# Zhijian-Mei/py-debruijn

Measured on AMD Instinct MI355X. Metric: k-mers/s hashed+graph-built at k=31, higher is better.
Workload: dtype u64

## Files before the change

py-debruijn_amd/_dbg.py:

```python
from __future__ import annotations

import ctypes as C
import os

import numpy as np

_HERE = os.path.dirname(os.path.abspath(__file__))
LIB_PATH = os.environ.get("DBG_LIB") or os.path.join(_HERE, "libdbg_hip.so")

DBG_OK, DBG_E_ARG, DBG_E_HIP, DBG_E_ALPHABET, DBG_E_CAPACITY, DBG_E_NOMEM = 0, -1, -2, -3, -4, -5
F_INDEG, F_KEEP_MASK, F_KEEP_SHIFT, F_BRANCH, F_PULLED = 0x01, 0x1E, 1, 0x20, 0x40
NO_NODE = 0xFFFFFFFF
ABI_VERSION = 6

SYMBOLS = (
    "dbg_create", "dbg_destroy", "dbg_last_error", "dbg_abi_version", "dbg_set_option", "dbg_set_reads", "dbg_set_reads_fasta",
    "dbg_set_reads_fasta_file", "dbg_fasta_ingest_stats", "dbg_set_reads_device",
    "dbg_synth_reads", "dbg_reads_checksum", "dbg_copy_reads", "dbg_reads_device", "dbg_build", "dbg_refine_edge_order", "dbg_export_orders",
    "dbg_get_alphabet", "dbg_export_keepmask", "dbg_export_dict_order",
    "dbg_prune", "dbg_remove_tips",
    "dbg_mark_pull_reads", "dbg_walk", "dbg_get_sizes", "dbg_get_stats", "dbg_get_counter", "dbg_export_nodes", "dbg_export_keys_hi",
    "dbg_export_succ",
    "dbg_export_csr", "dbg_export_pull_ranks", "dbg_export_pull_reads", "dbg_export_contigs",
    "dbg_export_contig_index", "dbg_export_contig_text", "dbg_device_views", "dbg_shard_extract", "dbg_shard_bucket_counts", "dbg_shard_record_layout", "dbg_shard_build", "dbg_shard_answer", "dbg_shard_apply",
    "dbg_import_graph", "dbg_device_keys_hi",
    "dbg_support_read_scores", "dbg_export_sorted_fasta", "dbg_build_multipass", "dbg_part_count", "dbg_part_sizes", "dbg_export_part", "dbg_part_device_views",
    "dbg_shard_build_multipass", "dbg_shard_build_multipass_from", "dbg_shard_extract_part", "dbg_part_queries", "dbg_part_answer", "dbg_part_apply", "dbg_multipass_finish",
    "dbg_export_marked", "dbg_part_keys_hi", "dbg_take_reads",
    "dbg_part_prune", "dbg_part_select", "dbg_part_gather", "dbg_part_mark", "dbg_part_clear", "dbg_part_cross_targets",
    "dbg_part_segments", "dbg_part_pflags", "dbg_scan_reads_for_keys", "dbg_set_orders", "dbg_part_segment_text",
    "dbg_build_from_walk", "dbg_build_from_walks",
)


class Sizes(C.Structure):
    _fields_ = [("k", C.c_int32), ("abi_version", C.c_int32)] + [
        (n, C.c_uint64) for n in (
            "n_reads", "n_bytes", "n_kmer_instances", "n_edge_instances", "table_capacity", "n_nodes", "n_edges",
            "n_branch", "n_pulled", "n_pull_reads", "n_starts", "n_contigs", "contig_chars", "tip_rounds",
            "contigs_materialised", "max_degree")]

    def as_dict(self):
        return {n: getattr(self, n) for n, _ in self._fields_}


class Stats(C.Structure):
    _fields_ = [(n, C.c_double) for n in (
        "ms_startbits", "ms_table_init", "ms_count", "ms_compact", "ms_succ", "ms_csr", "ms_build_total", "ms_prune",
        "ms_tips", "ms_pull_reads", "ms_walk", "ms_h2d", "ms_extract", "ms_partition")] + [
        (n, C.c_uint64) for n in ("count_launches", "n_records", "n_buckets", "n_queries")]

    def as_dict(self):
        return {n: getattr(self, n) for n, _ in self._fields_}


class IngestStats(C.Structure):
    _fields_ = [(n, C.c_uint64) for n in (
        "bytes_read", "chunks", "chunk_bytes", "peak_device_bytes", "n_reads", "n_bases")] + [
        (n, C.c_double) for n in ("ms_total", "ms_io_wait", "ms_h2d", "ms_parse")]

    def as_dict(self):
        return {n: getattr(self, n) for n, _ in self._fields_}


class WalkBlock(C.Structure):
    _fields_ = [("src", C.c_void_p), ("contigs", C.c_void_p), ("n", C.c_uint64)]


COUNTERS = ("extract_presplit_fallbacks", "extract_presplit_rehists", "resolve_direct_hits", "resolve_keyed")


class DbgError(RuntimeError):
    def __init__(self, code, msg):
        super().__init__(f"dbg error {code}: {msg}")
        self.code = code


class AlphabetError(DbgError, ValueError):
    pass


_lib = None


def load_library():
    global _lib
    if _lib is not None:
        return _lib
    if not os.path.exists(LIB_PATH):
        raise OSError(f"{LIB_PATH} not found: build it with py-debruijn_amd/csrc/build.sh "
                      f"(there is no CPU fallback for the device path)")
    try:
        import torch
    except ImportError:
        pass
    lib = C.CDLL(LIB_PATH)
    H = C.c_void_p
    u64p, u32p, u8p = C.POINTER(C.c_uint64), C.POINTER(C.c_uint32), C.POINTER(C.c_uint8)
    vp = C.c_void_p
    sig = {
        "dbg_create": (C.c_int, [C.c_int, C.POINTER(H)]),
        "dbg_destroy": (None, [H]),
        "dbg_last_error": (C.c_char_p, [H]),
        "dbg_abi_version": (C.c_int, []),
        "dbg_set_option": (C.c_int, [H, C.c_char_p, C.c_int64]),
        "dbg_set_reads": (C.c_int, [H, vp, vp, C.c_uint64]),
        "dbg_set_reads_fasta": (C.c_int, [H, vp, C.c_uint64]),
        "dbg_set_reads_fasta_file": (C.c_int, [H, C.c_char_p, C.c_uint64, C.c_uint64, C.c_uint64]),
        "dbg_fasta_ingest_stats": (C.c_int, [H, C.POINTER(IngestStats)]),
        "dbg_set_reads_device": (C.c_int, [H, vp, C.c_uint64, vp, C.c_uint64]),
        "dbg_synth_reads": (C.c_int, [H, C.c_uint64, C.c_uint64, C.c_uint64, C.c_uint64, C.c_uint32, C.c_uint32]),
        "dbg_reads_checksum": (C.c_int, [H, u64p]),
        "dbg_copy_reads": (C.c_int, [H, vp, vp]),
        "dbg_build": (C.c_int, [H, C.c_int, C.c_uint64]),
        "dbg_refine_edge_order": (C.c_int, [H]),
        "dbg_export_orders": (C.c_int, [H, vp, vp]),
        "dbg_get_alphabet": (C.c_int, [H, vp, C.POINTER(C.c_int), C.POINTER(C.c_int)]),
        "dbg_export_keepmask": (C.c_int, [H, vp]),
        "dbg_prune": (C.c_int, [H, C.c_double]),
        "dbg_remove_tips": (C.c_int, [H]),
        "dbg_mark_pull_reads": (C.c_int, [H]),
        "dbg_walk": (C.c_int, [H, C.c_int, C.c_uint64]),
        "dbg_get_sizes": (C.c_int, [H, C.POINTER(Sizes)]),
        "dbg_get_stats": (C.c_int, [H, C.POINTER(Stats)]),
        "dbg_get_counter": (C.c_int, [H, C.c_char_p, C.POINTER(C.c_uint64)]),
        "dbg_export_nodes": (C.c_int, [H, vp, vp, vp, vp]),
        "dbg_export_keys_hi": (C.c_int, [H, vp]),
        "dbg_export_dict_order": (C.c_int, [H, vp]),
        "dbg_export_succ": (C.c_int, [H, vp]),
        "dbg_export_csr": (C.c_int, [H, vp, vp, vp]),
        "dbg_export_pull_ranks": (C.c_int, [H, vp]),
        "dbg_export_pull_reads": (C.c_int, [H, vp]),
        "dbg_export_contigs": (C.c_int, [H, vp, vp, vp, vp, vp]),
        "dbg_export_contig_index": (C.c_int, [H, vp, vp, vp, vp]),
        "dbg_export_contig_text": (C.c_int, [H, C.c_uint64, vp, C.c_uint64]),
        "dbg_device_views": (C.c_int, [H] + [C.POINTER(vp)] * 5),
        "dbg_shard_extract": (C.c_int, [H, C.c_int, C.c_int, u64p, C.POINTER(vp), C.POINTER(vp), C.POINTER(vp)]),
        "dbg_shard_bucket_counts": (C.c_int, [H, u64p]),
        "dbg_shard_record_layout": (C.c_int, [H, C.POINTER(C.c_int), C.POINTER(C.c_int)]),
        "dbg_shard_build": (C.c_int, [H, C.c_int, C.c_int, C.c_int, vp, vp, vp, u64p, u64p, u64p, u64p, C.POINTER(vp), u64p, C.c_int]),
        "dbg_shard_answer": (C.c_int, [H, vp, C.c_uint64, vp]),
        "dbg_build_multipass": (C.c_int, [H, C.c_int, C.c_int]),
        "dbg_export_sorted_fasta": (C.c_int, [H, vp, vp, C.c_uint64, u64p]),
        "dbg_support_read_scores": (C.c_int, [H, vp, vp, C.c_uint64, vp, vp, vp, vp, C.c_uint64, vp, vp]),
        "dbg_part_count": (C.c_int, [H, C.POINTER(C.c_int)]),
        "dbg_shard_build_multipass": (C.c_int, [H, C.c_int, C.c_int, C.c_int, C.c_int, vp, vp, vp, C.c_int, u64p, u64p, u64p]),
        "dbg_shard_build_multipass_from": (C.c_int, [H, C.c_int, C.c_int, C.c_int, C.c_int, C.c_int, vp, vp, vp, C.c_int, u64p, u64p, u64p]),
        "dbg_shard_extract_part": (C.c_int, [H, C.c_int, C.c_int, C.c_int, C.c_int, u64p, C.POINTER(C.c_void_p), C.POINTER(C.c_void_p), C.POINTER(C.c_void_p)]),
        "dbg_part_queries": (C.c_int, [H, C.c_int, u64p, u64p, C.POINTER(vp)]),
        "dbg_part_answer": (C.c_int, [H, C.c_int, vp, C.c_uint64, vp]),
        "dbg_part_apply": (C.c_int, [H, C.c_int, C.c_int, vp]),
        "dbg_multipass_finish": (C.c_int, [H]),
# ... 650 lines not shown
```

py-debruijn_amd/csrc/dbg_hip.hip:

```cpp
#include <hip/hip_runtime.h>

#include <algorithm>
#include <chrono>
#include <cstdlib>
#include <cstdio>
#include <cstring>
#include <string>
#include <vector>

#include <cerrno>
#include <fcntl.h>
#include <sys/stat.h>
#include <unistd.h>

#include <rocprim/device/device_radix_sort.hpp>

#include "../../include/dbg.h"
#include "dbg_device.h"
#include "dbg_sk.h"
#include "dbg_sk2.h"
#include "dbg_sk3.h"
#include "dbg_wsk2.h"
#include "dbg_generic.h"
#include "dbg_genref.h"
// ... 58 lines not shown
    uint8_t *d_fsorder = nullptr;
    bool order_exact = false;
    uint32_t *d_succ = nullptr;
    bool nodes_in_arena = false;
    bool csr_built = false;
    uint64_t *d_rowptr = nullptr;
    uint32_t *d_col = nullptr, *d_ecnt = nullptr;
    bool dense_pending = false;
    uint32_t *d_rowptr32 = nullptr;
    void *d_stamps_st = nullptr;
    int stamps_st_bytes = 0;

    bool pruned = false, tipped = false;
    uint64_t n_branch = 0, n_pulled = 0, tip_rounds = 0;
    uint64_t *d_pull_rank = nullptr;

    uint8_t *d_read_flags = nullptr;
    uint64_t n_pull_reads = 0;
    bool pull_reads_done = false;

    uint64_t n_starts = 0, n_contigs = 0, contig_chars = 0;
    bool starts_known = false;
    struct { const uint64_t *w0 = nullptr, *w1 = nullptr; const void *st = nullptr; int st_bytes = 0;
             const uint64_t *b_start = nullptr, *b_cnt = nullptr; bool valid = false; } sk_src;
    uint64_t *d_ctg_off = nullptr;
    char *d_ctg_chars = nullptr;
    uint64_t *d_ctg_score = nullptr, *d_ctg_stamp = nullptr;
    uint32_t *d_ctg_seq = nullptr;
    uint32_t *d_ctg_start = nullptr;
    uint32_t *d_lift = nullptr;
    int lift_levels = 0;
    bool walked = false;
    bool walk_final = false;
    bool walk_indexed = false;
    uint64_t walk_jump_min = 1ull << 14;

    int D = 4, sym_bits = 2, n_sym = 0;
    bool alpha_known = false, is_dna = true;
    uint8_t alphabet[32] = {0};
    uint8_t *d_lut = nullptr;
    char *d_alpha = nullptr;
    uint32_t *d_keepmask = nullptr;
    uint8_t *d_rank_mc = nullptr, *d_rank_fs = nullptr;

    int engine = 0;
    int bucket_bits = 0;
    int lds_slots = 4096;
    int phase_limit = 0;
    int est_scale_pct = 100;
    int wide_engine = 1;
    int count_kernel_u64 = 3;
    int stamp64 = 0;
    int resolve_sorted = 0;
    int resolve_direct = 1;
    int resolve_count = 0;
    uint64_t resolve_direct_hits = 0, resolve_keyed = 0;
    int wcount_kernel = 2;
    int count_kernel = 2;

    struct Buf {
        void *p = nullptr;
        uint64_t bytes = 0;
    };
    Buf ar_rec[2][3], ar_q[2][3], ar_node[8], ar_misc[MISC_SLOTS], ar_csr[4], ar_dir, ar_l2, ar_scan, ar_shard[6], ar_walk[3], ar_wide[6], ar_refine[4], ar_tips[4], ar_part[4][3] ;
    int sk_T = 0, sk_l1 = 0, sk_l2 = 0, sk_nb2 = 0 , sk_cap = 0;
    bool refine_streaming = false;
    int target_distinct = 0;
    int shard_stamp64 = 0;
    int extract_generic = 0;
    int extract_presplit = DBG_EXTRACT_PRESPLIT;
    uint64_t presplit_rehists = 0;
    uint64_t presplit_fallbacks = 0;
    uint64_t sk_n_ranges = 0, sk_n_buckets = 0;
    SkGeom sk_geom{};
    void *shard_state = nullptr;
    void *multipass = nullptr;
    bool dropping_parts = false;
    dbg *spare_part = nullptr;
    bool wide_owner = false;
    bool borrowed_stream = false;
    bool arena_freed = false;
    std::vector<uint64_t> host_seg_cnt;
    std::vector<uint64_t> host_scpre;
    uint64_t shard_node_limit = 0;
    bool partial_graph = false;
    uint64_t *d_btab = nullptr;
    uint64_t btab_cap = 0;
    struct NkBlock {
        uint64_t n_src = 0, n_reads = 0;
        uint32_t *next = nullptr, *z = nullptr, *start = nullptr;
    };
    bool nk_graph = false;
    uint64_t nk_reads = 0, nk_bytes = 0;
    std::vector<NkBlock> nk_blocks;
    uint8_t *d_nk_read_flags = nullptr;

    dbg_stats_t stats{};
    dbg_ingest_stats_t ingest{};
};

struct ShardState {
    int n_shards = 0, my_shard = 0, shard_bits = 0, k = 0;
    std::vector<uint64_t> q_start, q_cnt;
    uint64_t n_remote = 0;
    uint64_t n_kmer_inst_local = 0;
    std::vector<uint64_t> l1_counts;
    int rec_words = 1, rec_stamp_bytes = 4;
};
static ShardState &shard_of(dbg *h);
static void multipass_free(dbg *h);
static void drop_spare_part(dbg *h);

static int buf_ensure(dbg *h, dbg::Buf &b, uint64_t bytes) {
    if (bytes == 0) bytes = 16;
    if (b.bytes >= bytes) return DBG_OK;
    if (b.p) { (void)hipFreeAsync(b.p, h->stream); h->arena_freed = true; }
    b.p = nullptr;
    b.bytes = 0;
    static const bool trace = getenv("DBG_TRACE_ALLOC") != nullptr;
    const auto t_alloc = std::chrono::steady_clock::now();
    hipError_t e = hipMallocAsync(&b.p, bytes, h->stream);
    if (trace) {
        const double ms = std::chrono::duration<double, std::milli>(std::chrono::steady_clock::now() - t_alloc).count();
        if (ms > 5.0) fprintf(stderr, "[dbg] hipMallocAsync(%.3f GB) took %.1f ms (buffer %p of handle %p)\n", bytes / 1e9, ms, (void *)&b, (void *)h);
    }
    if (e != hipSuccess) {
        (void)hipGetLastError();
        (void)hipStreamSynchronize(h->stream);
        hipMemPool_t pool;
        if (hipDeviceGetDefaultMemPool(&pool, h->device) == hipSuccess) (void)hipMemPoolTrimTo(pool, 0);
        e = hipMallocAsync(&b.p, bytes, h->stream);
    }
    if (e != hipSuccess) {
        (void)hipGetLastError();
        h->err = std::string("hipMallocAsync(") + std::to_string(bytes) + "): " + hipGetErrorString(e);
        b.p = nullptr;
        return DBG_E_NOMEM;
    }
    b.bytes = bytes;
    return DBG_OK;
}
static void buf_free(dbg *h, dbg::Buf &b) {
    if (b.p) { (void)hipFreeAsync(b.p, h->stream); h->arena_freed = true; }
    b.p = nullptr;
    b.bytes = 0;
}
static void pool_trim(dbg *h) {
    if (!h->arena_freed) return;
    (void)hipStreamSynchronize(h->stream);
    hipMemPool_t pool;
    if (hipDeviceGetDefaultMemPool(&pool, h->device) == hipSuccess) (void)hipMemPoolTrimTo(pool, 0);
    (void)hipGetLastError();
    h->arena_freed = false;
}

#define HIPCHK(h, call)                                                                      \
    do {                                                                                     \
        hipError_t e_ = (call);                                                              \
        if (e_ != hipSuccess) {                                                              \
            (h)->err = std::string(#call) + ": " + hipGetErrorString(e_);                    \
            return e_ == hipErrorOutOfMemory ? DBG_E_NOMEM : DBG_E_HIP;                      \
        }                                                                                    \
    } while (0)

#define CHK(expr)                 \
    do {                          \
        int rc_ = (expr);         \
        if (rc_ != DBG_OK) return rc_; \
    } while (0)

template <class T>
static int dev_alloc(dbg *h, T **p, uint64_t count) {
    *p = nullptr;
    if (count == 0) count = 1;
    HIPCHK(h, hipMalloc((void **)p, count * sizeof(T)));
    return DBG_OK;
}
template <class T>
static void dev_free(T *&p) {
    if (p) (void)hipFree(p);
    p = nullptr;
}

static inline unsigned grid_for(uint64_t n, unsigned block) { return (unsigned)((n + block - 1) / block); }

struct Timer {
    hipEvent_t a = nullptr, b = nullptr;
    hipStream_t s;
    explicit Timer(hipStream_t st) : s(st) {
        (void)hipEventCreate(&a);
        (void)hipEventCreate(&b);
        (void)hipEventRecord(a, s);
    }
    double stop() {
        (void)hipEventRecord(b, s);
        (void)hipEventSynchronize(b);
        float ms = 0;
        (void)hipEventElapsedTime(&ms, a, b);
        return ms;
    }
    ~Timer() {
        (void)hipEventDestroy(a);
        (void)hipEventDestroy(b);
    }
};

constexpr int SCAN_ITEMS = 16;
constexpr int SCAN_TILE = 256 * SCAN_ITEMS;

template <class F>
__global__ __launch_bounds__(256) void k_scan_reduce(uint64_t n, F f, uint64_t *partial) {
    uint64_t base = (uint64_t)blockIdx.x * SCAN_TILE + (uint64_t)threadIdx.x * SCAN_ITEMS;
    uint64_t s = 0;
#pragma unroll
    for (int i = 0; i < SCAN_ITEMS; ++i)
        if (base + i < n) s += f(base + i);
    uint64_t tot;
    (void)block_exscan_256(s, &tot);
    if (threadIdx.x == 0) partial[blockIdx.x] = tot;
}

__global__ __launch_bounds__(256) void k_scan_partials(uint64_t *partial, uint64_t nblk, uint64_t *total) {
    uint64_t carry = 0;
    for (uint64_t base = 0; base < nblk; base += 256) {
        uint64_t i = base + threadIdx.x;
        uint64_t v = i < nblk ? partial[i] : 0;
        uint64_t tot;
        uint64_t ex = block_exscan_256(v, &tot);
        if (i < nblk) partial[i] = carry + ex;
        carry += tot;
    }
    if (threadIdx.x == 0) *total = carry;
}

template <class F, class OutT>
__global__ __launch_bounds__(256) void k_scan_write(uint64_t n, F f, const uint64_t *partial, OutT *out) {
    uint64_t base = (uint64_t)blockIdx.x * SCAN_TILE + (uint64_t)threadIdx.x * SCAN_ITEMS;
    uint64_t v[SCAN_ITEMS];
    uint64_t s = 0;
#pragma unroll
    for (int i = 0; i < SCAN_ITEMS; ++i) {
        v[i] = (base + i < n) ? f(base + i) : 0;
        s += v[i];
    }
    uint64_t tot;
    uint64_t run = partial[blockIdx.x] + block_exscan_256(s, &tot);
#pragma unroll
    for (int i = 0; i < SCAN_ITEMS; ++i) {
        if (base + i < n) out[base + i] = (OutT)run;
        run += v[i];
    }
}

template <class F, class OutT>
static int exclusive_scan(dbg *h, uint64_t n, F f, OutT *out, uint64_t *h_total) {
    uint64_t nblk = (n + SCAN_TILE - 1) / SCAN_TILE;
    if (nblk == 0) nblk = 1;
    CHK(buf_ensure(h, h->ar_scan, (nblk + 1) * 8));
    uint64_t *partial = (uint64_t *)h->ar_scan.p;
    uint64_t *d_total = partial + nblk;
    hipLaunchKernelGGL(HIP_KERNEL_NAME(k_scan_reduce<F>), dim3((unsigned)nblk), dim3(256), 0, h->stream, n, f, partial);
    hipLaunchKernelGGL(k_scan_partials, dim3(1), dim3(256), 0, h->stream, partial, nblk, d_total);
    hipLaunchKernelGGL(HIP_KERNEL_NAME(k_scan_write<F, OutT>), dim3((unsigned)nblk), dim3(256), 0, h->stream, n, f,
                       partial, out);
    if (!h_total) return DBG_OK;
    hipError_t e = hipMemcpyAsync(h_total, d_total, 8, hipMemcpyDeviceToHost, h->stream);
    if (e == hipSuccess) e = hipStreamSynchronize(h->stream);
    if (e != hipSuccess) {
        h->err = std::string("exclusive_scan: ") + hipGetErrorString(e);
        return DBG_E_HIP;
    }
    return DBG_OK;
}

template <class F>
static int reduce_sum(dbg *h, uint64_t n, F f, uint64_t *h_total) {
    uint64_t nblk = (n + SCAN_TILE - 1) / SCAN_TILE;
    if (nblk == 0) nblk = 1;
    CHK(buf_ensure(h, h->ar_scan, (nblk + 1) * 8));
    uint64_t *partial = (uint64_t *)h->ar_scan.p;
    hipLaunchKernelGGL(HIP_KERNEL_NAME(k_scan_reduce<F>), dim3((unsigned)nblk), dim3(256), 0, h->stream, n, f, partial);
    hipLaunchKernelGGL(k_scan_partials, dim3(1), dim3(256), 0, h->stream, partial, nblk, partial + nblk);
    hipError_t e = hipMemcpyAsync(h_total, partial + nblk, 8, hipMemcpyDeviceToHost, h->stream);
    if (e == hipSuccess) e = hipStreamSynchronize(h->stream);
    if (e != hipSuccess) {
        h->err = std::string("reduce_sum: ") + hipGetErrorString(e);
        return DBG_E_HIP;
    }
// ... 1026 lines not shown
                                                   uint64_t n_nodes, int levels, char *chars) {
    const uint64_t c = (uint64_t)blockIdx.x * blockDim.x + threadIdx.x;
    if (c >= n_chars) return;
    uint64_t lo = 0, hi = n_ctg;
    while (hi - lo > 1) {
        const uint64_t mid = (lo + hi) >> 1;
        if (ctg_off[mid] <= c) lo = mid; else hi = mid;
    }
    const uint64_t j = c - ctg_off[lo];
    uint32_t x = ctg_start[lo];
    if (j < (uint64_t)g.k) { chars[c] = g.char_at(x, (int)j); return; }
    uint64_t d = j - (uint64_t)g.k + 1;
    for (int l = 0; l < levels && d; ++l, d >>= 1)
        if (d & 1) x = up[(uint64_t)l * n_nodes + x];
    chars[c] = g.sym_char(g.last_code(x));
}

static const char *const kPartialGraph =
    "this handle holds one shard of a multi-GPU build: gather the shards first (multi_gpu.gather_graph / dbg_import_graph)";
static int nk_mark_contigs(dbg *h);
static void free_build(dbg *h) {
    multipass_free(h);
    dev_free(h->d_tab); dev_free(h->d_occ);
    if (h->nodes_in_arena) {
        h->d_keys = nullptr; h->d_stamps = nullptr; h->d_cnt = nullptr; h->d_flags = nullptr;
        h->d_order = nullptr; h->d_succ = nullptr; h->d_deg = nullptr; h->d_keys_hi = nullptr;
        h->nodes_in_arena = false;
    }
    dev_free(h->d_btab);
    h->btab_cap = 0;
    dev_free(h->d_keys_hi);
    dev_free(h->d_fsorder);
    h->order_exact = false;
    dev_free(h->d_keepmask); dev_free(h->d_rank_mc); dev_free(h->d_rank_fs);
    h->D = 4; h->sym_bits = 2;
    dev_free(h->d_keys); dev_free(h->d_stamps); dev_free(h->d_cnt); dev_free(h->d_flags);
    dev_free(h->d_order); dev_free(h->d_succ); dev_free(h->d_deg);
    h->d_rowptr = nullptr; h->d_col = nullptr; h->d_ecnt = nullptr;
    h->d_rowptr32 = nullptr; h->d_stamps_st = nullptr; h->stamps_st_bytes = 0;
    h->dense_pending = false;
    h->csr_built = false;
    h->d_pull_rank = nullptr;
    dev_free(h->d_read_flags);
    dev_free(h->d_ctg_off); dev_free(h->d_ctg_chars); dev_free(h->d_ctg_score); dev_free(h->d_ctg_stamp);
    dev_free(h->d_ctg_seq); dev_free(h->d_ctg_start); dev_free(h->d_lift);
    h->lift_levels = 0;
    h->partial_graph = false;
    h->sk_src.valid = false;
    h->k = 0; h->cap = 0; h->n_nodes = h->n_edges = 0;
    h->pruned = h->tipped = h->pull_reads_done = h->walked = h->walk_indexed = false;
    h->n_branch = h->n_pulled = h->tip_rounds = h->n_pull_reads = 0;
    h->n_starts = h->n_contigs = h->contig_chars = 0;
    h->starts_known = false;
    h->n_kmer_inst = h->n_edge_inst = 0;
    for (auto &b : h->nk_blocks) { dev_free(b.next); dev_free(b.z); dev_free(b.start); }
    h->nk_blocks.clear();
    dev_free(h->d_nk_read_flags);
    h->nk_graph = false;
    h->nk_reads = h->nk_bytes = 0;
}

static void free_reads(dbg *h) {
    if (h->own_bases) dev_free(h->d_bases);
    if (h->own_offsets) dev_free(h->d_offsets);
    h->d_bases = nullptr; h->d_offsets = nullptr;
    h->own_bases = h->own_offsets = false;
    dev_free(h->d_startbits);
    dev_free(h->d_lut); dev_free(h->d_alpha);
    h->alpha_known = false;
    h->n_bytes = h->n_reads = 0;
}

extern "C" int dbg_abi_version(void) { return DBG_ABI_VERSION; }

extern "C" int dbg_create(int device, dbg_t **out) {
    if (!out) return DBG_E_ARG;
    *out = nullptr;
    int n = 0;
    if (hipGetDeviceCount(&n) != hipSuccess || device < 0 || device >= n) return DBG_E_HIP;
    dbg *h = new (std::nothrow) dbg();
    if (!h) return DBG_E_NOMEM;
    h->device = device;
    if (hipSetDevice(device) != hipSuccess || hipStreamCreate(&h->stream) != hipSuccess ||
        hipMalloc((void **)&h->d_scalars, 128 * sizeof(uint64_t)) != hipSuccess) {
        delete h;
        return DBG_E_HIP;
    }
    {
        hipMemPool_t pool;
        if (hipDeviceGetDefaultMemPool(&pool, device) == hipSuccess) {
            uint64_t keep = ~0ull;
            (void)hipMemPoolSetAttribute(pool, hipMemPoolAttrReleaseThreshold, &keep);
        }
        (void)hipGetLastError();
    }
    *out = h;
    return DBG_OK;
}

extern "C" void dbg_destroy(dbg_t *h) {
    if (!h) return;
    (void)hipSetDevice(h->device);
    (void)hipStreamSynchronize(h->stream);
    h->dropping_parts = true;
    free_build(h);
    if (h->spare_part) { dbg_destroy(h->spare_part); h->spare_part = nullptr; }
    free_reads(h);
    for (auto &lvl : h->ar_rec) for (auto &b : lvl) buf_free(h, b);
    for (auto &lvl : h->ar_q) for (auto &b : lvl) buf_free(h, b);
    for (auto &b : h->ar_node) buf_free(h, b);
    for (auto &b : h->ar_misc) buf_free(h, b);
    for (auto &b : h->ar_csr) buf_free(h, b);
    buf_free(h, h->ar_dir);
    buf_free(h, h->ar_l2);
    for (auto &b : h->ar_shard) buf_free(h, b);
    for (auto &b : h->ar_walk) buf_free(h, b);
    for (auto &b : h->ar_wide) buf_free(h, b);
    for (auto &b : h->ar_refine) buf_free(h, b);
    for (auto &b : h->ar_tips) buf_free(h, b);
    for (auto &lvl : h->ar_part) for (auto &b : lvl) buf_free(h, b);
    buf_free(h, h->ar_scan);
    dev_free(h->d_scalars);
    delete (ShardState *)h->shard_state;
    (void)hipStreamSynchronize(h->stream);
    if (!h->borrowed_stream) (void)hipStreamDestroy(h->stream);
    delete h;
}

extern "C" const char *dbg_last_error(const dbg_t *h) { return h ? h->err.c_str() : "null handle"; }

static int make_startbits(dbg *h) {
    Timer t(h->stream);
    dev_free(h->d_startbits);
    h->startbits_words = (h->n_bytes + 1 + 31) / 32 + SB_WORDS + 2;
    CHK(dev_alloc(h, &h->d_startbits, h->startbits_words));
    HIPCHK(h, hipMemsetAsync(h->d_startbits, 0, h->startbits_words * 4, h->stream));
    hipLaunchKernelGGL(k_startbits, dim3(grid_for(h->n_reads + 1, 256)), dim3(256), 0, h->stream, h->d_offsets,
                       h->n_reads, h->d_startbits);
    HIPCHK(h, hipGetLastError());
    h->stats.ms_startbits = t.stop();
    return DBG_OK;
}

extern "C" int dbg_set_reads(dbg_t *h, const char *bases, const uint64_t *offsets, uint64_t n_reads) {
    if (!h || !offsets || (n_reads && !bases && offsets[n_reads] != 0)) return DBG_E_ARG;
    HIPCHK(h, hipSetDevice(h->device));
    if (offsets[0] != 0) { h->err = "offsets[0] must be 0"; return DBG_E_ARG; }
    for (uint64_t i = 0; i < n_reads; ++i)
        if (offsets[i + 1] < offsets[i]) { h->err = "offsets must be non-decreasing"; return DBG_E_ARG; }
    free_build(h);
    free_reads(h);
    const uint64_t nb = offsets[n_reads];
    Timer t(h->stream);
    CHK(dev_alloc(h, &h->d_bases, nb + 64));
    h->own_bases = true;
    CHK(dev_alloc(h, &h->d_offsets, n_reads + 1));
    h->own_offsets = true;
    if (nb) HIPCHK(h, hipMemcpyAsync(h->d_bases, bases, nb, hipMemcpyHostToDevice, h->stream));
    HIPCHK(h, hipMemcpyAsync(h->d_offsets, offsets, (n_reads + 1) * 8, hipMemcpyHostToDevice, h->stream));
    h->stats.ms_h2d = t.stop();
    h->n_bytes = nb;
    h->n_reads = n_reads;
    return make_startbits(h);
}

extern "C" int dbg_set_reads_fasta(dbg_t *h, const char *text, uint64_t n_text) {
    if (!h || (n_text && !text)) return DBG_E_ARG;
    HIPCHK(h, hipSetDevice(h->device));
    free_build(h);
    free_reads(h);
    char *d_text = nullptr;
    uint32_t *bits = nullptr, *word_rank = nullptr, *len = nullptr;
    uint64_t *line_start = nullptr, *read_idx = nullptr, *byte_off = nullptr;
    uint8_t *is_read = nullptr;
    auto cleanup = [&]() {
        dev_free(d_text); dev_free(bits); dev_free(word_rank); dev_free(len); dev_free(line_start); dev_free(read_idx);
        dev_free(byte_off); dev_free(is_read);
    };
    int rc = DBG_OK;
    uint64_t n_lines = 0, n_reads = 0, n_bases = 0;
    do {
        Timer t(h->stream);
        if ((rc = dev_alloc(h, &d_text, n_text + 64)) != DBG_OK) break;
        if (n_text && hipMemcpyAsync(d_text, text, n_text, hipMemcpyHostToDevice, h->stream) != hipSuccess) { h->err = "H2D copy failed"; rc = DBG_E_HIP; break; }
        h->stats.ms_h2d = t.stop();
        const uint64_t n_words = (n_text + 31) / 32;
        if ((rc = dev_alloc(h, &bits, n_words)) != DBG_OK) break;
        if ((rc = dev_alloc(h, &word_rank, n_words)) != DBG_OK) break;
        if (n_words) {
            hipLaunchKernelGGL(k_fa_mark, dim3(grid_for(n_words, 256)), dim3(256), 0, h->stream, d_text, n_text, bits);
            if ((rc = exclusive_scan(h, n_words, PopcWords{bits}, word_rank, &n_lines)) != DBG_OK) break;
        }
        if ((rc = dev_alloc(h, &line_start, n_lines)) != DBG_OK) break;
        if ((rc = dev_alloc(h, &is_read, n_lines)) != DBG_OK) break;
        if ((rc = dev_alloc(h, &len, n_lines)) != DBG_OK) break;
        if ((rc = dev_alloc(h, &read_idx, n_lines)) != DBG_OK) break;
        if ((rc = dev_alloc(h, &byte_off, n_lines)) != DBG_OK) break;
        if (n_lines) {
            hipLaunchKernelGGL(k_fa_line_starts, dim3(grid_for(n_words, 256)), dim3(256), 0, h->stream, bits, word_rank, n_words,
                               line_start);
            hipLaunchKernelGGL(k_fa_lines, dim3(grid_for(n_lines, 256)), dim3(256), 0, h->stream, d_text, n_text, line_start,
                               n_lines, is_read, len);
            if ((rc = exclusive_scan(h, n_lines, ByteSet{is_read}, read_idx, &n_reads)) != DBG_OK) break;
            if ((rc = exclusive_scan(h, n_lines, U32At{len}, byte_off, &n_bases)) != DBG_OK) break;
        }
        if ((rc = dev_alloc(h, &h->d_bases, n_bases + 64)) != DBG_OK) break;
        h->own_bases = true;
// ... 600 lines not shown
    uint32_t *occ = nullptr, *eocc = nullptr, *word_rank = nullptr;
    unsigned long long *estamp = nullptr;
    auto cleanup = [&]() { dev_free(nodes); dev_free(edges); dev_free(occ); dev_free(eocc); dev_free(word_rank); dev_free(estamp); };
    int rc = DBG_OK;
    do {
        if ((rc = dev_alloc(h, &nodes, cap)) != DBG_OK) break;
        if ((rc = dev_alloc(h, &edges, cap)) != DBG_OK) break;
        if ((rc = dev_alloc(h, &occ, cap / 32)) != DBG_OK) break;
        if ((rc = dev_alloc(h, &eocc, cap / 32)) != DBG_OK) break;
        (void)hipMemsetAsync(occ, 0, cap / 8, h->stream);
        (void)hipMemsetAsync(eocc, 0, cap / 8, h->stream);
        (void)hipMemsetAsync(h->d_scalars, 0, 64 * 8, h->stream);
        hipLaunchKernelGGL(k_g_init_tables, dim3(grid_for(cap, 256)), dim3(256), 0, h->stream, nodes, edges, cap);
        if (h->n_bytes) {
            const unsigned grid = (unsigned)std::min<uint64_t>((h->n_bytes + 255) / 256, 1u << 16);
            hipLaunchKernelGGL(k_g_insert, dim3(grid), dim3(256), 0, h->stream, h->d_bases, h->n_bytes, h->d_startbits, k,
                               h->d_lut, nodes, occ, edges, eocc, cap - 1, (unsigned long long *)h->d_scalars);
        }
        uint64_t sc[4] = {0, 0, 0, 0};
        if (hipMemcpyAsync(sc, h->d_scalars, 32, hipMemcpyDeviceToHost, h->stream) != hipSuccess ||
            hipStreamSynchronize(h->stream) != hipSuccess) { h->err = "generic count failed"; rc = DBG_E_HIP; break; }
        if (sc[0] & STATUS_TABLE_FULL) { h->err = "generic engine: hash table full"; rc = DBG_E_CAPACITY; break; }
        h->n_kmer_inst = sc[1];
        h->n_edge_inst = sc[2];
        h->stats.ms_count = t_count.stop();
        h->stats.count_launches = 1;
        Timer t_c(h->stream);
        const uint64_t n_words = cap / 32;
        if ((rc = dev_alloc(h, &word_rank, n_words)) != DBG_OK) break;
        uint64_t n = 0;
        if ((rc = exclusive_scan(h, n_words, PopcWords{occ}, word_rank, &n)) != DBG_OK) break;
        h->n_nodes = n;
        if ((rc = dev_alloc(h, &h->d_keys, n)) != DBG_OK) break;
        if ((rc = dev_alloc(h, &h->d_stamps, n)) != DBG_OK) break;
        if ((rc = dev_alloc(h, &h->d_flags, n)) != DBG_OK) break;
        if ((rc = dev_alloc(h, &h->d_cnt, n * GEN_D)) != DBG_OK) break;
        if ((rc = dev_alloc(h, &h->d_succ, n * GEN_D)) != DBG_OK) break;
        if ((rc = dev_alloc(h, &h->d_deg, n)) != DBG_OK) break;
        if ((rc = dev_alloc(h, &h->d_keepmask, n)) != DBG_OK) break;
        if ((rc = dev_alloc(h, &h->d_rank_mc, n * GEN_D)) != DBG_OK) break;
        if ((rc = dev_alloc(h, &h->d_rank_fs, n * GEN_D)) != DBG_OK) break;
        if ((rc = dev_alloc(h, &estamp, n * GEN_D)) != DBG_OK) break;
        if (n) {
            (void)hipMemsetAsync(h->d_cnt, 0, n * GEN_D * 4, h->stream);
            (void)hipMemsetAsync(h->d_succ, 0xFF, n * GEN_D * 4, h->stream);
            (void)hipMemsetAsync(estamp, 0xFF, n * GEN_D * 8, h->stream);
            (void)hipMemsetAsync(h->d_keepmask, 0, n * 4, h->stream);
            hipLaunchKernelGGL(k_g_gather, dim3(grid_for(n_words, 256)), dim3(256), 0, h->stream, nodes, occ, word_rank, n_words,
                               h->d_keys, h->d_stamps, h->d_flags);
            hipLaunchKernelGGL(k_g_edges, dim3(grid_for(cap, 256)), dim3(256), 0, h->stream, edges, cap, nodes, cap - 1, k,
                               h->d_cnt, h->d_succ, estamp, (unsigned long long *)h->d_scalars);
            hipLaunchKernelGGL(k_g_rank, dim3(grid_for(n, 256)), dim3(256), 0, h->stream, n, h->d_cnt, estamp, h->d_rank_mc,
                               h->d_rank_fs, h->d_deg);
        }
        if (hipMemcpyAsync(sc, h->d_scalars, 8, hipMemcpyDeviceToHost, h->stream) != hipSuccess ||
            hipStreamSynchronize(h->stream) != hipSuccess) { h->err = "generic graph assembly failed"; rc = DBG_E_HIP; break; }
        if (sc[0] & STATUS_SUCC_MISSING) { h->err = "internal: edge endpoint missing from the node table"; rc = DBG_E_HIP; break; }
        h->stats.ms_succ = t_c.stop();
        h->order_exact = true;
    } while (0);
    cleanup();
    return rc;
}

extern "C" int dbg_set_option(dbg_t *h, const char *name, int64_t value) {
    if (!h || !name) return DBG_E_ARG;
    const std::string n(name);
    if (n == "engine" && (value == 0 || value == 1)) { h->engine = (int)value; return DBG_OK; }
    if (n == "bucket_bits" && value >= 0 && value <= SK_BUCKET_BITS) { h->bucket_bits = (int)value; return DBG_OK; }
    if (n == "lds_slots" && (value == 2048 || value == 4096)) { h->lds_slots = (int)value; return DBG_OK; }
    if (n == "phase_limit" && value >= 0 && value <= 5) { h->phase_limit = (int)value; return DBG_OK; }
    if (n == "estimate_scale_pct" && value >= 1 && value <= 1000) { h->est_scale_pct = (int)value; return DBG_OK; }
    if (n == "target_distinct" && value >= 0 && value <= 4096) { h->target_distinct = (int)value; return DBG_OK; }
    if (n == "shard_stamp64" && (value == 0 || value == 1)) { h->shard_stamp64 = (int)value; return DBG_OK; }
    if (n == "extract_generic" && (value == 0 || value == 1)) { h->extract_generic = (int)value; return DBG_OK; }
    if (n == "extract_presplit" && value >= 0 && value <= SK_PS_MAX_F0) { h->extract_presplit = (int)value; return DBG_OK; }
    if (n == "refine_streaming" && (value == 0 || value == 1)) { h->refine_streaming = value != 0; return DBG_OK; }
    if (n == "walk_jump_min_nodes" && value >= 0) { h->walk_jump_min = (uint64_t)value; return DBG_OK; }
    if (n == "wide_engine" && (value == 0 || value == 1)) { h->wide_engine = (int)value; return DBG_OK; }
    if (n == "count_kernel" && value >= 1 && value <= 3) { h->count_kernel = (int)value; return DBG_OK; }
    if (n == "stamp64" && (value == 0 || value == 1)) { h->stamp64 = (int)value; return DBG_OK; }
    if (n == "resolve_sorted" && value >= 0 && value <= 2) { h->resolve_sorted = (int)value; return DBG_OK; }
    if (n == "resolve_direct" && (value == 0 || value == 1)) { h->resolve_direct = (int)value; return DBG_OK; }
    if (n == "resolve_count" && (value == 0 || value == 1)) { h->resolve_count = (int)value; return DBG_OK; }
    if (n == "wcount_kernel" && (value == 1 || value == 2)) { h->wcount_kernel = (int)value; return DBG_OK; }
    if (n == "count_kernel_u64" && value >= 1 && value <= 3) { h->count_kernel_u64 = (int)value; return DBG_OK; }
    if (n == "shard_node_limit" && value >= 0 && value < (1ll << 29)) { h->shard_node_limit = (uint64_t)value; return DBG_OK; }
    h->err = "unknown option or value out of range: " + n;
    return DBG_E_ARG;
}

static int build_wide_once(dbg *h, int k, uint64_t table_capacity_hint, bool packed, bool *overflow) {
    if (h->n_bytes >= (1ull << 43)) { h->err = "reads too large for the 44-bit positions of the table's protocol word"; return DBG_E_CAPACITY; }
    uint64_t want = table_capacity_hint;
    if (!want) {
        uint64_t inst = 0;
        CHK(reduce_sum(h, h->n_reads, KmerInstances{h->d_offsets, (uint64_t)k}, &inst));
        want = (uint64_t)((double)(inst + 1) / 0.7);
    }
    const uint64_t cap = std::max<uint64_t>(1024, (want + 1023) / 1024 * 1024);
    const uint64_t pk_words = (h->n_bytes + 31) / 32, n_occ = cap / 32;
    uint64_t *pk = nullptr;
    WSlot *tab = nullptr;
    uint32_t *tcnt = nullptr, *word_rank = nullptr;
    uint8_t *occ = nullptr;
    auto cleanup = [&]() {};
    int rc = DBG_OK;
    uint64_t sc[4] = {0, 0, 0, 0};
    do {
        Timer t(h->stream);
        if ((rc = buf_ensure(h, h->ar_wide[0], (pk_words + 3) * 8)) != DBG_OK) break;
        if ((rc = buf_ensure(h, h->ar_wide[1], cap * sizeof(WSlot))) != DBG_OK) break;
        if (!packed && (rc = buf_ensure(h, h->ar_wide[2], cap * 16)) != DBG_OK) break;
        if ((rc = buf_ensure(h, h->ar_wide[3], cap)) != DBG_OK) break;
        if ((rc = buf_ensure(h, h->ar_wide[4], n_occ * 4)) != DBG_OK) break;
        pk = (uint64_t *)h->ar_wide[0].p;
        tab = (WSlot *)h->ar_wide[1].p;
        tcnt = packed ? nullptr : (uint32_t *)h->ar_wide[2].p;
        occ = (uint8_t *)h->ar_wide[3].p;
        word_rank = (uint32_t *)h->ar_wide[4].p;
        (void)hipMemsetAsync(pk + pk_words, 0, 3 * 8, h->stream);
        hipLaunchKernelGGL(k_wtab_init, dim3(grid_for(cap, 256)), dim3(256), 0, h->stream, tab, cap);
        if (tcnt) (void)hipMemsetAsync(tcnt, 0, cap * 16, h->stream);
        (void)hipMemsetAsync(occ, 0, cap, h->stream);
        (void)hipMemsetAsync(h->d_scalars, 0, 64 * 8, h->stream);
        if (pk_words)
            hipLaunchKernelGGL(k_wpack, dim3(grid_for(pk_words, 256)), dim3(256), 0, h->stream, h->d_bases, h->n_bytes,
                               pk_words, pk);
        h->stats.ms_table_init = t.stop();
        Timer tc(h->stream);
        const uint64_t tiles = (h->n_bytes + TILE - 1) / TILE;
        if (tiles)
            hipLaunchKernelGGL(k_wcount, dim3((unsigned)tiles), dim3(256), 0, h->stream, h->d_bases, h->n_bytes,
                               h->d_startbits, k, pk, tab, tcnt, cap, occ, (unsigned long long *)h->d_scalars);
        h->stats.count_launches = tiles ? 1 : 0;
        hipError_t e = hipMemcpyAsync(sc, h->d_scalars, 32, hipMemcpyDeviceToHost, h->stream);
        h->stats.ms_count = tc.stop();
        if (e != hipSuccess || hipGetLastError() != hipSuccess) { h->err = "k_wcount failed"; rc = DBG_E_HIP; break; }
        if (sc[0] & STATUS_BAD_BASE) { h->err = "reads hold a byte outside ACGT"; rc = DBG_E_ALPHABET; break; }
        if (sc[0] & STATUS_TABLE_FULL) { h->err = "hash table capacity exceeded"; rc = DBG_E_CAPACITY; break; }
        if (sc[0] & STATUS_WIDE_COUNTER16) { *overflow = true; rc = DBG_E_CAPACITY; h->err = "successor counter overflow"; break; }
        h->n_kmer_inst = sc[1];
        h->n_edge_inst = sc[2];

        Timer tg(h->stream);
        uint64_t total = 0;
        if ((rc = exclusive_scan(h, n_occ, OccBytes32{occ}, word_rank, &total)) != DBG_OK) break;
        if (total >= 0xFFFFFFFFull) { h->err = "more than 2^32-1 nodes"; rc = DBG_E_CAPACITY; break; }
        h->n_nodes = total;
        if ((rc = buf_ensure(h, h->ar_node[0], total * 8)) != DBG_OK) break;
        if ((rc = buf_ensure(h, h->ar_node[1], total * 8)) != DBG_OK) break;
        if ((rc = buf_ensure(h, h->ar_node[2], total * 16)) != DBG_OK) break;
        if ((rc = buf_ensure(h, h->ar_node[3], total)) != DBG_OK) break;
        if ((rc = buf_ensure(h, h->ar_node[4], total)) != DBG_OK) break;
        if ((rc = buf_ensure(h, h->ar_node[5], total * 16)) != DBG_OK) break;
        if ((rc = buf_ensure(h, h->ar_node[6], total)) != DBG_OK) break;
        if ((rc = buf_ensure(h, h->ar_wide[5], total * 8)) != DBG_OK) break;
        h->d_keys = (uint64_t *)h->ar_node[0].p;
        h->d_stamps = (uint64_t *)h->ar_node[1].p;
        h->d_cnt = (uint32_t *)h->ar_node[2].p;
        h->d_flags = (uint8_t *)h->ar_node[3].p;
        h->d_order = (uint8_t *)h->ar_node[4].p;
        h->d_succ = (uint32_t *)h->ar_node[5].p;
        h->d_deg = (uint8_t *)h->ar_node[6].p;
        h->d_keys_hi = (uint64_t *)h->ar_wide[5].p;
        h->nodes_in_arena = true;
// ... 717 lines not shown
                               base_chr, per_score, h->d_stamps, h->d_ctg_off, h->d_ctg_score, h->d_ctg_stamp, h->d_ctg_seq,
                               ctg_start);
            hipError_t e = hipStreamSynchronize(h->stream);
            if (e != hipSuccess) { h->err = std::string("walk index: ") + hipGetErrorString(e); rc = DBG_E_HIP; break; }
            h->walk_indexed = true;
            if (n_chr > max_chars) break;
            const uint64_t longest = h->n_nodes + (uint64_t)h->k;
            int levels = 1;
            while ((1ull << levels) <= longest) ++levels;
            if (n_ctg && (uint64_t)levels * h->n_nodes * 4 <= (8ull << 30)) {
                if ((rc = dev_alloc(h, &h->d_ctg_chars, n_chr)) != DBG_OK) break;
                if ((rc = dev_alloc(h, &lift, (uint64_t)levels * h->n_nodes)) != DBG_OK) break;
                const dim3 ngrid(grid_for(h->n_nodes, 256));
                hipLaunchKernelGGL(HIP_KERNEL_NAME(k_lift_init<G>), ngrid, dim3(256), 0, h->stream, h->n_nodes, g, lift);
                for (int l = 1; l < levels; ++l)
                    hipLaunchKernelGGL(k_lift_step, ngrid, dim3(256), 0, h->stream, h->n_nodes, lift + (uint64_t)(l - 1) * h->n_nodes,
                                       lift + (uint64_t)l * h->n_nodes);
                hipLaunchKernelGGL(HIP_KERNEL_NAME(k_text_fill<G>), dim3(grid_for(n_chr, 256)), dim3(256), 0, h->stream, n_chr, g,
                                   h->d_ctg_off, n_ctg, ctg_start, lift, h->n_nodes, levels, h->d_ctg_chars);
                text_done = true;
            }
        }
        if (!text_done) {
            if ((rc = dev_alloc(h, &h->d_ctg_chars, n_chr)) != DBG_OK) break;
            launch(1);
        }
        if (hipGetLastError() != hipSuccess) { h->err = "walk pass 1 launch failed"; rc = DBG_E_HIP; break; }
        hipError_t e = hipStreamSynchronize(h->stream);
        if (e != hipSuccess) { h->err = std::string("walk: ") + hipGetErrorString(e); rc = DBG_E_HIP; break; }
        h->walked = true;
        h->walk_indexed = true;
    } while (0);
    cleanup();
    h->stats.ms_walk = t.stop();
    return rc;
}

extern "C" int dbg_walk(dbg_t *h, int final_mode, uint64_t max_chars) {
    if (!h || !h->pruned) { if (h) h->err = "dbg_prune must run first"; return DBG_E_ARG; }
    HIPCHK(h, hipSetDevice(h->device));
    if (h->D == GEN_D) return walk_impl(h, gen_view(h), final_mode, max_chars);
    return walk_impl(h, dna_view(h), final_mode, max_chars);
}

extern "C" int dbg_get_sizes(dbg_t *h, dbg_sizes_t *o) {
    if (!h || !o) return DBG_E_ARG;
    if (h->k && h->n_nodes && !h->starts_known) {
        HIPCHK(h, hipSetDevice(h->device));
        CHK(ensure_starts(h));
    }
    memset(o, 0, sizeof(*o));
    o->k = h->k;
    o->abi_version = DBG_ABI_VERSION;
    o->n_reads = h->n_reads + h->nk_reads;
    o->n_bytes = h->n_bytes + h->nk_bytes;
    o->n_kmer_instances = h->n_kmer_inst;
    o->n_edge_instances = h->n_edge_inst;
    o->table_capacity = h->cap;
    o->n_nodes = h->n_nodes;
    o->n_edges = h->n_edges;
    o->n_branch = h->n_branch;
    o->n_pulled = h->n_pulled;
    o->n_pull_reads = h->n_pull_reads;
    o->n_starts = h->n_starts;
    o->n_contigs = h->n_contigs;
    o->contig_chars = h->contig_chars;
    o->tip_rounds = h->tip_rounds;
    o->contigs_materialised = h->walked ? 1 : 0;
    o->max_degree = (uint64_t)h->D;
    return DBG_OK;
}

extern "C" int dbg_get_stats(dbg_t *h, dbg_stats_t *o) {
    if (!h || !o) return DBG_E_ARG;
    *o = h->stats;
    return DBG_OK;
}

extern "C" int dbg_get_counter(dbg_t *h, const char *name, uint64_t *out) {
    if (!h || !name || !out) return DBG_E_ARG;
    const std::string n(name);
    if (n == "extract_presplit_rehists") { *out = h->presplit_rehists; return DBG_OK; }
    if (n == "extract_presplit_fallbacks") { *out = h->presplit_fallbacks; return DBG_OK; }
    if (n == "resolve_direct_hits") { *out = h->resolve_direct_hits; return DBG_OK; }
    if (n == "resolve_keyed") { *out = h->resolve_keyed; return DBG_OK; }
    h->err = "unknown counter: " + n;
    return DBG_E_ARG;
}

#define D2H(h, dst, src, bytes)                                                                       do {                                                                                                  if ((dst) && (bytes)) HIPCHK(h, hipMemcpyAsync((dst), (src), (bytes), hipMemcpyDeviceToHost, (h)->stream));     } while (0)

extern "C" int dbg_export_nodes(dbg_t *h, uint64_t *keys, uint64_t *stamps, uint32_t *counts, uint8_t *flags) {
    if (!h || !h->k) return DBG_E_ARG;
    HIPCHK(h, hipSetDevice(h->device));
    CHK(ensure_dense(h));
    if (keys && !h->d_keys) memset(keys, 0, h->n_nodes * 8);
    else D2H(h, keys, h->d_keys, h->n_nodes * 8);
    D2H(h, stamps, h->d_stamps, h->n_nodes * 8);
    D2H(h, counts, h->d_cnt, h->n_nodes * 4 * h->D);
    D2H(h, flags, h->d_flags, h->n_nodes);
    HIPCHK(h, hipStreamSynchronize(h->stream));
    return DBG_OK;
}

extern "C" int dbg_export_keys_hi(dbg_t *h, uint64_t *keys_hi) {
    if (!h || !h->k || !keys_hi) return DBG_E_ARG;
    HIPCHK(h, hipSetDevice(h->device));
    if (!h->d_keys_hi) {
        memset(keys_hi, 0, h->n_nodes * 8);
        return DBG_OK;
    }
    D2H(h, keys_hi, h->d_keys_hi, h->n_nodes * 8);
    HIPCHK(h, hipStreamSynchronize(h->stream));
    return DBG_OK;
}

extern "C" int dbg_export_succ(dbg_t *h, uint32_t *succ) {
    if (!h || !h->k) return DBG_E_ARG;
    HIPCHK(h, hipSetDevice(h->device));
    CHK(ensure_dense(h));
    D2H(h, succ, h->d_succ, h->n_nodes * 4 * h->D);
    HIPCHK(h, hipStreamSynchronize(h->stream));
    return DBG_OK;
}

extern "C" int dbg_export_csr(dbg_t *h, uint64_t *row_ptr, uint32_t *col, uint32_t *cnt) {
    if (!h || !h->k) return DBG_E_ARG;
    HIPCHK(h, hipSetDevice(h->device));
    CHK(ensure_dense(h));
    D2H(h, row_ptr, h->d_rowptr, (h->n_nodes + 1) * 8);
    D2H(h, col, h->d_col, h->n_edges * 4);
    D2H(h, cnt, h->d_ecnt, h->n_edges * 4);
    HIPCHK(h, hipStreamSynchronize(h->stream));
    return DBG_OK;
}

extern "C" int dbg_export_pull_ranks(dbg_t *h, uint64_t *ranks) {
    if (!h || !h->tipped) { if (h) h->err = "dbg_remove_tips must run first"; return DBG_E_ARG; }
    HIPCHK(h, hipSetDevice(h->device));
    D2H(h, ranks, h->d_pull_rank, h->n_nodes * 8);
    HIPCHK(h, hipStreamSynchronize(h->stream));
    return DBG_OK;
}

extern "C" int dbg_export_pull_reads(dbg_t *h, uint8_t *read_flags) {
    if (!h || !h->pull_reads_done) { if (h) h->err = "dbg_mark_pull_reads must run first"; return DBG_E_ARG; }
    HIPCHK(h, hipSetDevice(h->device));
    if (h->nk_graph) {
        D2H(h, read_flags, h->d_nk_read_flags, h->nk_reads);
        if (read_flags) read_flags += h->nk_reads;
    }
    D2H(h, read_flags, h->d_read_flags, h->n_reads);
    HIPCHK(h, hipStreamSynchronize(h->stream));
    return DBG_OK;
}

extern "C" int dbg_export_contig_index(dbg_t *h, uint64_t *offsets, uint64_t *scores, uint64_t *start_stamp,
                                       uint32_t *seq_in_start) {
    if (!h || !h->walk_indexed) { if (h) h->err = "dbg_walk must run first"; return DBG_E_ARG; }
    HIPCHK(h, hipSetDevice(h->device));
    D2H(h, offsets, h->d_ctg_off, (h->n_contigs + 1) * 8);
    D2H(h, scores, h->d_ctg_score, h->n_contigs * 8);
    D2H(h, start_stamp, h->d_ctg_stamp, h->n_contigs * 8);
    D2H(h, seq_in_start, h->d_ctg_seq, h->n_contigs * 4);
    HIPCHK(h, hipStreamSynchronize(h->stream));
    return DBG_OK;
// ... 55 lines not shown
    if (len) hipLaunchKernelGGL(HIP_KERNEL_NAME(k_text_one<G>), dim3(grid_for(len, 256)), dim3(256), 0, h->stream, g, start, len,
                                h->d_lift, h->n_nodes, h->lift_levels, tmp);
    hipError_t e = len ? hipMemcpyAsync(buf, tmp, len, hipMemcpyDeviceToHost, h->stream) : hipSuccess;
    if (e == hipSuccess) e = hipStreamSynchronize(h->stream);
    dev_free(tmp);
    if (e != hipSuccess) { h->err = std::string("contig text: ") + hipGetErrorString(e); return DBG_E_HIP; }
    return DBG_OK;
}

extern "C" int dbg_export_contig_text(dbg_t *h, uint64_t index, char *buf, uint64_t buf_len) {
    if (!h || !h->walk_indexed || !buf) { if (h) h->err = "dbg_walk must run first"; return DBG_E_ARG; }
    if (index >= h->n_contigs) { h->err = "contig index out of range"; return DBG_E_ARG; }
    HIPCHK(h, hipSetDevice(h->device));
    if (h->walked) {
        uint64_t off[2];
        HIPCHK(h, hipMemcpyAsync(off, h->d_ctg_off + index, 16, hipMemcpyDeviceToHost, h->stream));
        HIPCHK(h, hipStreamSynchronize(h->stream));
        if (buf_len < off[1] - off[0]) { h->err = "buffer smaller than the contig"; return DBG_E_ARG; }
        if (off[1] > off[0]) HIPCHK(h, hipMemcpyAsync(buf, h->d_ctg_chars + off[0], off[1] - off[0], hipMemcpyDeviceToHost, h->stream));
        HIPCHK(h, hipStreamSynchronize(h->stream));
        return DBG_OK;
    }
    if (!h->d_ctg_start) { h->err = "no per-contig start nodes (walk did not take the list-ranking path)"; return DBG_E_ARG; }
    if (h->D == GEN_D) return contig_text_impl(h, gen_view(h), index, buf, buf_len);
    return contig_text_impl(h, dna_view(h), index, buf, buf_len);
}

#ifdef DBG_MS_PROF
extern "C" int dbg_debug_ms_prof(unsigned long long *out8, int reset) {
    if (hipMemcpyFromSymbol(out8, HIP_SYMBOL(dbgk::g_ms_prof), 64) != hipSuccess) return DBG_E_HIP;
    if (reset) { unsigned long long z[8] = {}; if (hipMemcpyToSymbol(HIP_SYMBOL(dbgk::g_ms_prof), z, 64) != hipSuccess) return DBG_E_HIP; }
    return DBG_OK;
}
#endif

#ifdef DBG_CNT_PROF
extern "C" int dbg_debug_cnt_prof(unsigned long long *out32, int reset) {
    if (hipMemcpyFromSymbol(out32, HIP_SYMBOL(dbgk::g_cnt_prof), 512) != hipSuccess) return DBG_E_HIP;
    if (reset) { unsigned long long z[64] = {}; if (hipMemcpyToSymbol(HIP_SYMBOL(dbgk::g_cnt_prof), z, 512) != hipSuccess) return DBG_E_HIP; }
    return DBG_OK;
}
#endif

extern "C" int dbg_device_keys_hi(dbg_t *h, const void **d_keys_hi) {
    if (!h || !h->k || !d_keys_hi) return DBG_E_ARG;
    *d_keys_hi = h->d_keys_hi;
    return DBG_OK;
}

extern "C" int dbg_reads_device(dbg_t *h, const void **d_bases, uint64_t *n_bytes, const void **d_offsets, uint64_t *n_reads) {
    if (!h || !h->d_offsets) { if (h) h->err = "no reads set"; return DBG_E_ARG; }
    if (d_bases) *d_bases = h->d_bases;
    if (n_bytes) *n_bytes = h->n_bytes;
    if (d_offsets) *d_offsets = h->d_offsets;
    if (n_reads) *n_reads = h->n_reads;
    return DBG_OK;
}

extern "C" int dbg_device_views(dbg_t *h, const void **d_keys, const void **d_counts, const void **d_stamps,
                                const void **d_flags, const void **d_succ) {
    if (!h || !h->k) return DBG_E_ARG;
    HIPCHK(h, hipSetDevice(h->device));
    CHK(ensure_dense(h));
    if (d_keys) *d_keys = h->d_keys;
    if (d_counts) *d_counts = h->d_cnt;
    if (d_stamps) *d_stamps = h->d_stamps;
    if (d_flags) *d_flags = h->d_flags;
    if (d_succ) *d_succ = h->d_succ;
    return DBG_OK;
}

struct CeilDiv {
    const uint64_t *cnt;
    uint64_t d;
    __device__ uint64_t operator()(uint64_t i) const { return (cnt[i] + d - 1) / d; }
};

template <class ST, bool HAS_ST, class STI = ST, int STHI = 0>
static int multisplit_level(dbg *h, const uint64_t *p_start, const uint64_t *p_cnt, uint32_t n_seg, uint32_t spg,
                            uint64_t total, const uint64_t *in_w0, const uint64_t *in_w1, const STI *in_st,
                            uint64_t *out_w0, uint64_t *out_w1, ST *out_st, int shift, int nb, uint64_t *c_start,
                            uint64_t *c_cnt, dbg::Buf &b_scpre, dbg::Buf &b_cmat, dbg::Buf &b_offs, int fbits = 0,
                            const uint64_t *seg_add = nullptr, unsigned long long *d_sums = nullptr,
                            const uint64_t *host_cnt = nullptr, const uint32_t *ready_cmat = nullptr) {
    CHK(buf_ensure(h, b_scpre, (uint64_t)(n_seg + 1) * 8));
    uint64_t *sc_pre = (uint64_t *)b_scpre.p;
    uint64_t nsc = 0;
    if (ready_cmat) {
        std::vector<uint64_t> &pre = h->host_scpre;
        pre.resize((size_t)n_seg + 1);
        for (uint32_t i = 0; i <= n_seg; ++i) pre[i] = i;
        nsc = n_seg;
        HIPCHK(h, hipMemcpyAsync(sc_pre, pre.data(), pre.size() * 8, hipMemcpyHostToDevice, h->stream));
    } else if (host_cnt) {
        std::vector<uint64_t> &pre = h->host_scpre;
        pre.resize((size_t)n_seg + 1);
        for (uint32_t i = 0; i < n_seg; ++i) { pre[i] = nsc; nsc += (host_cnt[i] + MS_SC - 1) / MS_SC; }
        pre[n_seg] = nsc;
        HIPCHK(h, hipMemcpyAsync(sc_pre, pre.data(), pre.size() * 8, hipMemcpyHostToDevice, h->stream));
    } else {
        CHK(exclusive_scan(h, n_seg, CeilDiv{p_cnt, (uint64_t)MS_SC}, sc_pre, &nsc));
        HIPCHK(h, hipMemcpyAsync(sc_pre + n_seg, &nsc, 8, hipMemcpyHostToDevice, h->stream));
    }
    MsParents P{p_start, p_cnt, sc_pre, n_seg, spg};
    const uint64_t n_log = nsc * (uint64_t)nb;
    if (!ready_cmat) CHK(buf_ensure(h, b_cmat, n_log * 4));
    CHK(buf_ensure(h, b_offs, n_log * 8));
    const uint32_t *cmat = ready_cmat ? ready_cmat : (const uint32_t *)b_cmat.p;
    uint64_t *offs = (uint64_t *)b_offs.p;
    if (nsc) {
        if (ready_cmat)
            ;
        else if (d_sums)
            hipLaunchKernelGGL(HIP_KERNEL_NAME(k_ms_hist<true>), dim3((unsigned)nsc), dim3(256), 0, h->stream, P, in_w1, shift, nb,
                               fbits, (uint32_t *)b_cmat.p, d_sums);
        else
            hipLaunchKernelGGL(HIP_KERNEL_NAME(k_ms_hist<false>), dim3((unsigned)nsc), dim3(256), 0, h->stream, P, in_w1, shift, nb,
                               fbits, (uint32_t *)b_cmat.p, (unsigned long long *)nullptr);
        HIPCHK(h, hipGetLastError());
        CHK(exclusive_scan(h, n_log, MsLogical{P, cmat, nb}, offs, (uint64_t *)nullptr));
    }
    const uint64_t n_child = (uint64_t)(n_seg / spg) * nb;
    hipLaunchKernelGGL(k_ms_children, dim3(grid_for(n_child, 256)), dim3(256), 0, h->stream, P, offs, nb, total, c_start,
                       c_cnt);
    if (nsc) {
        auto kern = k_ms_scatter<ST, HAS_ST, STI, STHI>;
        const size_t lds = sizeof(MsLds<ST>);
        HIPCHK(h, hipFuncSetAttribute((const void *)kern, hipFuncAttributeMaxDynamicSharedMemorySize, (int)lds));
        hipLaunchKernelGGL(kern, dim3((unsigned)nsc), dim3(MS_NT), lds, h->stream, P, in_w0, in_w1, in_st, seg_add, shift, nb,
                           fbits, offs, out_w0, out_w1, out_st);
    }
    HIPCHK(h, hipGetLastError());
    return DBG_OK;
}

static void sk_provisional_bits(const dbg *h, uint64_t n_inst, double own, double target, int shard_bits, bool presplit_senders,
                                int l1_wide_from, int *T_out, int *l1_out) {
    constexpr int T_MAX = 20;
    int T = h->bucket_bits;
    if (T == 0) {
        const double want = (double)n_inst * own * 0.4 / target;
        while (T < T_MAX && (double)(1ull << T) < want) ++T;
    }
    if (T < shard_bits) T = shard_bits;
    if (presplit_senders) T = std::max(9, T);
    *T_out = T;
    *l1_out = T < 9 ? T : (T >= l1_wide_from && !presplit_senders ? 10 : 9);
}

template <int CAP> constexpr double SK_TARGET_DISTINCT = CAP * 0.36;

struct ExtractSplit {
    double target = 0.0;
    int f0 = 0;
    uint32_t n_wg = 0;
    int l1 = 0;
    const uint32_t *cmat = nullptr;
};

template <class ST>
static int sk_extract(dbg *h, int k, uint64_t *w0[2], uint64_t *w1[2], ST *st[2], uint64_t **seg_start_out,
                      uint64_t **seg_cnt_out, uint32_t *n_seg_out, uint64_t *n_rec_out, int part = 0, int n_parts = 1,
                      ExtractSplit *xs = nullptr) {
    const int m = sk_m_for_k(k), w = k - m + 1;
    unsigned long long *sc_dev = (unsigned long long *)h->d_scalars;
    const uint64_t all_tiles = (h->n_bytes + TILE - 1) / TILE;
    const uint64_t tile_first = all_tiles * (uint64_t)part / (uint64_t)n_parts;
    const uint64_t tiles = all_tiles * (uint64_t)(part + 1) / (uint64_t)n_parts - tile_first;
    uint64_t sc[8] = {0};
    uint32_t n_wg = (uint32_t)std::min<uint64_t>(std::max<uint64_t>(tiles, 1), 2048);
    uint64_t tiles_per_wg = (tiles + n_wg - 1) / n_wg;
    const double density = std::min(1.0, 2.6 / (double)(w + 1) + 1.3 * (double)(h->n_reads + 1) / (double)(h->n_bytes + 1) + 0.01);
    uint64_t seg_cap = (w == 1) ? tiles_per_wg * TILE : (uint64_t)((double)(tiles_per_wg * TILE) * density) + 256;
    int f0 = (xs && n_parts == 1 && tiles && m == SK_MAX_M && w <= 19 && !h->extract_generic) ? h->extract_presplit : 0;
    constexpr double PS_SLACK = 1.5;
    const uint32_t n_wg_plain = n_wg;
    const uint64_t seg_cap_plain = seg_cap;
    uint64_t n_seg = n_wg;
    int ps_l1 = 0;
    if (f0) {
        const uint64_t F0 = 1ull << f0;
        const double per_tile = (w == 1 ? 1.0 : density) * TILE * PS_SLACK / (double)F0;
        const uint64_t tpw_max = std::max<uint64_t>(1, (uint64_t)((double)(MS_SC - 64) / per_tile));
        int n_cu = 0;
        HIPCHK(h, hipDeviceGetAttribute(&n_cu, hipDeviceAttributeMultiprocessorCount, h->device));
        n_wg = (uint32_t)std::max<uint64_t>(std::min<uint64_t>(tiles, (uint64_t)n_cu * DBG_PS_WG_PER_CU), (tiles + tpw_max - 1) / tpw_max);
        tiles_per_wg = (tiles + n_wg - 1) / n_wg;
        seg_cap = std::min<uint64_t>(MS_SC, (uint64_t)((double)tiles_per_wg * per_tile) + 64);
        n_seg = (uint64_t)n_wg * F0;
        const uint64_t cut = h->n_reads * (uint64_t)(k - 1);
        int T_guess = 0;
        sk_provisional_bits(h, h->n_bytes > cut ? h->n_bytes - cut : 0, 1.0, xs->target, 0, false, DBG_L1_WIDE_FROM, &T_guess, &ps_l1);
        if (ps_l1 < f0) ps_l1 = 0;
    }
    std::vector<uint64_t> hseg;
    uint64_t *seg_start = nullptr, *seg_cnt = nullptr, *seg_nk = nullptr, *seg_ne = nullptr;
    uint32_t *ps_cmat = nullptr;
    uint64_t n_rec = 0;
    Timer t(h->stream);
    for (int attempt = 0; attempt < 3; ++attempt) {
        CHK(buf_ensure(h, h->ar_misc[MISC_SEGMENTS], (n_seg * 2 + (uint64_t)n_wg * 2) * 8));
        seg_start = (uint64_t *)h->ar_misc[MISC_SEGMENTS].p; seg_cnt = seg_start + n_seg; seg_nk = seg_cnt + n_seg; seg_ne = seg_nk + n_wg;
        hseg.assign((size_t)(n_seg * 2 + (uint64_t)n_wg * 2), 0);
        if (f0 && ps_l1) {
            CHK(buf_ensure(h, h->ar_misc[MISC_MS_CMAT], n_seg * 4 << (ps_l1 - f0)));
            ps_cmat = (uint32_t *)h->ar_misc[MISC_MS_CMAT].p;
        }
        const uint64_t rec_cap = seg_cap * n_seg;
        for (int set = 0; set < 2; ++set) {
            CHK(buf_ensure(h, h->ar_rec[set][0], rec_cap * 8));
            CHK(buf_ensure(h, h->ar_rec[set][1], rec_cap * 8));
            CHK(buf_ensure(h, h->ar_rec[set][2], rec_cap * sizeof(ST)));
            w0[set] = (uint64_t *)h->ar_rec[set][0].p;
            w1[set] = (uint64_t *)h->ar_rec[set][1].p;
            st[set] = (ST *)h->ar_rec[set][2].p;
        }
        for (uint64_t g = 0; g < n_seg; ++g) hseg[g] = g * seg_cap;
        HIPCHK(h, hipMemcpyAsync(seg_start, hseg.data(), (size_t)n_seg * 8, hipMemcpyHostToDevice, h->stream));
        HIPCHK(h, hipMemsetAsync(seg_cnt, 0, (size_t)(n_seg + (uint64_t)n_wg * 2) * 8, h->stream));
        HIPCHK(h, hipMemsetAsync(h->d_scalars, 0, 64 * 8, h->stream));
        if (tiles) {
            bool launched = false;
            if (m == SK_MAX_M && !h->extract_generic) {
#define DBG_EXW_CASE(W_) case W_: \
                if (f0) hipLaunchKernelGGL(HIP_KERNEL_NAME(k_sk_extract_w<ST, W_, true>), dim3(n_wg), dim3(256), 0, h->stream, \
                                           h->d_bases, h->n_bytes, h->d_startbits, tiles, w0[0], w1[0], st[0], seg_cap, seg_cnt, \
                                           seg_nk, seg_ne, sc_dev, tile_first, f0, ps_l1, ps_l1 ? ps_cmat : (uint32_t *)nullptr); \
                else hipLaunchKernelGGL(HIP_KERNEL_NAME(k_sk_extract_w<ST, W_, false>), dim3(n_wg), dim3(256), 0, h->stream, \
                                        h->d_bases, h->n_bytes, h->d_startbits, tiles, w0[0], w1[0], st[0], seg_cap, seg_cnt, \
                                        seg_nk, seg_ne, sc_dev, tile_first, 0, 0, (uint32_t *)nullptr); \
                launched = true; break;
                switch (w) {
                    DBG_EXW_CASE(1) DBG_EXW_CASE(2) DBG_EXW_CASE(3) DBG_EXW_CASE(4) DBG_EXW_CASE(5) DBG_EXW_CASE(6) DBG_EXW_CASE(7)
                    DBG_EXW_CASE(8) DBG_EXW_CASE(9) DBG_EXW_CASE(10) DBG_EXW_CASE(11) DBG_EXW_CASE(12) DBG_EXW_CASE(13)
                    DBG_EXW_CASE(14) DBG_EXW_CASE(15) DBG_EXW_CASE(16) DBG_EXW_CASE(17) DBG_EXW_CASE(18) DBG_EXW_CASE(19)
                    default: break;
                }
#undef DBG_EXW_CASE
            }
            if (!launched)
                hipLaunchKernelGGL(HIP_KERNEL_NAME(k_sk_extract<ST>), dim3(n_wg), dim3(256), 0, h->stream, h->d_bases,
                                   h->n_bytes, h->d_startbits, k, m, tiles, w0[0], w1[0], st[0], seg_cap, seg_cnt, seg_nk,
                                   seg_ne, sc_dev, tile_first);
            HIPCHK(h, hipGetLastError());
        }
        HIPCHK(h, hipMemcpyAsync(sc, h->d_scalars, 8, hipMemcpyDeviceToHost, h->stream));
        HIPCHK(h, hipMemcpyAsync(hseg.data() + n_seg, seg_cnt, (size_t)(n_seg + (uint64_t)n_wg * 2) * 8, hipMemcpyDeviceToHost,
                                 h->stream));
        HIPCHK(h, hipStreamSynchronize(h->stream));
        if (sc[0] & STATUS_BAD_BASE) { h->err = "reads hold a byte outside ACGT"; return DBG_E_ALPHABET; }
        if (!(sc[0] & STATUS_SEGMENT_FULL)) break;
        if (f0) {
            f0 = 0; ps_l1 = 0; ps_cmat = nullptr;
            ++h->presplit_fallbacks;
            n_wg = n_wg_plain; n_seg = n_wg;
            tiles_per_wg = (tiles + n_wg - 1) / n_wg;
            seg_cap = seg_cap_plain;
            continue;
        }
        if (seg_cap == tiles_per_wg * TILE) { h->err = "super-k-mer record buffer overflow"; return DBG_E_CAPACITY; }
        seg_cap = tiles_per_wg * TILE;
    }
    h->n_kmer_inst = h->n_edge_inst = 0;
    for (uint64_t g = 0; g < n_seg; ++g) n_rec += hseg[n_seg + g];
    for (uint32_t g = 0; g < n_wg; ++g) {
        h->n_kmer_inst += hseg[2 * n_seg + g];
        h->n_edge_inst += hseg[2 * n_seg + n_wg + g];
    }
    h->stats.ms_extract = t.stop();
    h->stats.n_records = n_rec;
    h->host_seg_cnt.assign(hseg.begin() + n_seg, hseg.begin() + 2 * (size_t)n_seg);
    if (xs) { xs->f0 = f0; xs->n_wg = n_wg; xs->l1 = ps_l1; xs->cmat = ps_l1 ? ps_cmat : nullptr; }
    *seg_start_out = seg_start;
    *seg_cnt_out = seg_cnt;
    *n_seg_out = (uint32_t)n_seg;
    *n_rec_out = n_rec;
    return DBG_OK;
}


struct Presplit {
    int n_senders = 0;
    const uint64_t *counts = nullptr;
    const uint64_t *recv_off = nullptr;
    const uint64_t *stamp_add = nullptr;
    const void *in_st = nullptr;
};

template <class Est>
struct SkPartitionParams {
    double target;
    int l1_wide_from;
    bool probe_first_owned;
    bool sum_instances;
    Est estimate;
};

struct SkPartition {
    uint64_t *b_start = nullptr, *b_cnt = nullptr;
    uint64_t n_buckets = 0;
    int where = 0;
    int l1 = 0, nb2 = 1, fb2 = 0, l2_pow = 0, nb3 = 1, fb3 = 0;
    double est_distinct = 0.0;
    uint64_t n_inst = 0, n_edge_inst = 0;
};

template <class ST, class STI, int STHI, class Est>
static int sk_partition(dbg *h, const SkPartitionParams<Est> &pp, const uint64_t *seg_start, const uint64_t *seg_cnt,
                        uint32_t n_seg, const uint64_t *host_cnt, const Presplit *pre, const ExtractSplit *xs, const uint64_t *in_w0,
                        const uint64_t *in_w1, const ST *in_st, uint64_t *w0[2], uint64_t *w1[2], ST *st[2], int shard_bits,
                        int my_shard, uint64_t n_rec, uint64_t n_inst, uint64_t n_edge_inst, SkPartition *out) {
    const double own = shard_bits ? (double)(1 << shard_bits) : 1.0;
    const bool auto_T = (h->bucket_bits == 0);
    int T = 0, l1 = 0;
    sk_provisional_bits(h, n_inst, own, pp.target, shard_bits, pre != nullptr, pp.l1_wide_from, &T, &l1);
    int l2 = std::min(10, T - l1);
    int nb2 = 0;
    int nb3 = (T - l1 - l2) > 0 ? 1 << (T - l1 - l2) : 1;
    const int nb1 = 1 << l1;
    CHK(buf_ensure(h, h->ar_misc[MISC_L1_CHILDREN], (uint64_t)nb1 * 16));
    uint64_t *c1_start = (uint64_t *)h->ar_misc[MISC_L1_CHILDREN].p, *c1_cnt = c1_start + nb1;
    dbg::Buf &ms_scpre = h->ar_misc[MISC_MS_SCPRE], &ms_cmat = h->ar_misc[MISC_MS_CMAT], &ms_offs = h->ar_misc[MISC_MS_OFFS];
    int where = 0;
    double est_distinct = 0.0;
    const int top = 6 + SK_BUCKET_BITS;
    Timer t_part(h->stream);
    const int bps = pre ? nb1 >> shard_bits : 0;
    const uint64_t b_lo = pre ? (uint64_t)my_shard * bps : 0;
    uint64_t *ps_start = nullptr, *ps_cnt = nullptr, *ps_add = nullptr;
    uint32_t ps_n = 0;
    if (pre) {
        ps_n = (uint32_t)(bps * pre->n_senders);
        std::vector<uint64_t> &hs = h->host_scpre;
        hs.assign((size_t)ps_n * 3, 0);
        for (int r = 0; r < pre->n_senders; ++r) {
            uint64_t at = pre->recv_off[r];
            for (int b = 0; b < bps; ++b) {
                const size_t i = (size_t)b * pre->n_senders + r;
                hs[i] = at;
                hs[ps_n + i] = pre->counts[(size_t)r * bps + b];
                hs[2 * (size_t)ps_n + i] = pre->stamp_add[r];
                at += pre->counts[(size_t)r * bps + b];
            }
        }
        CHK(buf_ensure(h, h->ar_misc[MISC_SEGMENTS], (uint64_t)ps_n * 3 * 8));
        ps_start = (uint64_t *)h->ar_misc[MISC_SEGMENTS].p; ps_cnt = ps_start + ps_n; ps_add = ps_cnt + ps_n;
        HIPCHK(h, hipMemcpyAsync(ps_start, hs.data(), hs.size() * 8, hipMemcpyHostToDevice, h->stream));
        HIPCHK(h, hipStreamSynchronize(h->stream));
    } else {
        if (xs && xs->f0 && l1 >= xs->f0) {
            if (xs->l1 != l1) ++h->presplit_rehists;
            CHK((multisplit_level<ST, true>(h, seg_start, seg_cnt, n_seg, xs->n_wg, n_rec, in_w0, in_w1, in_st, w0[1], w1[1], st[1],
                                            top - l1, nb1 >> xs->f0, c1_start, c1_cnt, ms_scpre, ms_cmat, ms_offs, 0, nullptr, nullptr,
                                            host_cnt, xs->l1 == l1 ? xs->cmat : nullptr)));
        } else {
            CHK((multisplit_level<ST, true>(h, seg_start, seg_cnt, n_seg, n_seg, n_rec, in_w0, in_w1, in_st, w0[1], w1[1], st[1],
                                            top - l1, nb1, c1_start, c1_cnt, ms_scpre, ms_cmat, ms_offs, 0, nullptr, nullptr, host_cnt)));
        }
        where = 1;
    }
    if (auto_T && l1 >= 9 && n_rec) {
        const uint32_t probe_bucket = (pp.probe_first_owned && shard_bits) ? (uint32_t)my_shard << (l1 - shard_bits) : 0u;
        const uint64_t inst_bucket = (uint64_t)((double)n_inst * own / nb1) * 2 + 1024;
        uint64_t set_cap = 1024;
        while (set_cap < inst_bucket * 2) set_cap <<= 1;
        CHK(buf_ensure(h, h->ar_misc[MISC_ESTIMATE_SET], set_cap * 8));
        unsigned long long *set = (unsigned long long *)h->ar_misc[MISC_ESTIMATE_SET].p;
        unsigned long long *d_est = (unsigned long long *)(h->d_scalars + SC_ESTIMATE);
        HIPCHK(h, hipMemsetAsync(set, 0xFF, set_cap * 8, h->stream));
        HIPCHK(h, hipMemsetAsync(d_est, 0, 16, h->stream));
        if (pre) {
            for (int r = 0; r < pre->n_senders; ++r) pp.estimate(128u, ps_start, ps_cnt, (uint32_t)r, in_w0, in_w1, set, set_cap - 1, d_est);
        } else {
            pp.estimate(512u, c1_start, c1_cnt, probe_bucket, w0[1], w1[1], set, set_cap - 1, d_est);
        }
        uint64_t est[2] = {0, 0};
        HIPCHK(h, hipMemcpyAsync(est, d_est, 16, hipMemcpyDeviceToHost, h->stream));
        HIPCHK(h, hipStreamSynchronize(h->stream));
        if (est[0]) {
            double distinct = (double)n_inst * own * (double)est[1] / (double)est[0];
            if (pre) {
                uint64_t probe_recs = 0;
                for (int r = 0; r < pre->n_senders; ++r) probe_recs += pre->counts[(size_t)r * bps];
                distinct = probe_recs ? (double)est[1] * (double)n_rec / (double)probe_recs * own : 0.0;
            }
            est_distinct = distinct / own;
            const double want = distinct / ((double)h->target_distinct > 0 ? (double)h->target_distinct : pp.target);
            const double want2 = std::max<double>(1.0, std::ceil(want / nb1));
            if (want2 <= 1024.0) {
                nb2 = (int)want2;
                nb3 = 1;
            } else {
                nb2 = 1024;
                nb3 = (int)std::min<double>((double)(1 << (SK_BUCKET_BITS - l1 - 10)), std::ceil(want2 / 1024.0));
            }
            l2 = nb2 > 1 ? 1 : 0;
        }
    }
    if (nb2 == 0 && l2 > 0) nb2 = 1 << l2;
    if (pre && l2 == 0) { l2 = 1; nb2 = 1; }
    if (l2 == 0) nb3 = 1;
    const int fb2 = (nb3 == 1 && ((nb2 > 0 && (nb2 & (nb2 - 1)) != 0) || (auto_T && l1 >= 9 && nb2 > 1))) ? SK_BUCKET_BITS - l1 : 0;
    const uint64_t n_l2 = l2 > 0 ? (uint64_t)nb1 * (uint64_t)nb2 : (uint64_t)nb1;
    const uint64_t n_buckets = n_l2 * (uint64_t)nb3;
    const int l2_pow = (fb2 || l2 == 0) ? 0 : (int)std::lround(std::log2((double)nb2));
    const int fb3 = nb3 > 1 ? SK_BUCKET_BITS - l1 - l2_pow : 0;
    CHK(buf_ensure(h, h->ar_misc[MISC_BUCKETS], n_buckets * 16));
    uint64_t *b_start = (uint64_t *)h->ar_misc[MISC_BUCKETS].p, *b_cnt = b_start + n_buckets;
    uint64_t *l2_start = b_start, *l2_cnt = b_cnt;
    if (nb3 > 1) {
        CHK(buf_ensure(h, h->ar_l2, n_l2 * 16));
        l2_start = (uint64_t *)h->ar_l2.p;
        l2_cnt = l2_start + n_l2;
    }
    if (l2 > 0) {
        const int sh2 = fb2 ? top - SK_BUCKET_BITS : top - l1 - l2_pow;
        if (pre) {
            unsigned long long *d_sums = (unsigned long long *)(h->d_scalars + SC_L2_SUMS);
            HIPCHK(h, hipMemsetAsync(b_start, 0, n_buckets * 16, h->stream));
            if (nb3 > 1) HIPCHK(h, hipMemsetAsync(l2_start, 0, n_l2 * 16, h->stream));
            HIPCHK(h, hipMemsetAsync(d_sums, 0, 16, h->stream));
            CHK((multisplit_level<ST, true, STI, STHI>(h, ps_start, ps_cnt, ps_n, (uint32_t)pre->n_senders, n_rec, in_w0, in_w1,
                                                       (const STI *)pre->in_st, w0[0], w1[0], st[0], sh2, nb2, l2_start + b_lo * nb2,
                                                       l2_cnt + b_lo * nb2, ms_scpre, ms_cmat, ms_offs, fb2, ps_add,
                                                       pp.sum_instances ? d_sums : (unsigned long long *)nullptr)));
            if (pp.sum_instances) {
                uint64_t sums[2] = {0, 0};
                HIPCHK(h, hipMemcpyAsync(sums, d_sums, 16, hipMemcpyDeviceToHost, h->stream));
                HIPCHK(h, hipStreamSynchronize(h->stream));
                n_inst = sums[0];
                n_edge_inst = sums[1];
                h->n_kmer_inst = n_inst;
                h->n_edge_inst = n_edge_inst;
            }
        } else {
            CHK((multisplit_level<ST, true>(h, c1_start, c1_cnt, (uint32_t)nb1, 1, n_rec, w0[1], w1[1], st[1], w0[0], w1[0],
                                            st[0], sh2, nb2, l2_start, l2_cnt, ms_scpre, ms_cmat, ms_offs, fb2)));
        }
        where = 0;
        if (nb3 > 1) {
            if (!w0[1]) {
                CHK(buf_ensure(h, h->ar_rec[1][0], (n_rec + 16) * 8));
                CHK(buf_ensure(h, h->ar_rec[1][1], (n_rec + 16) * 8));
                CHK(buf_ensure(h, h->ar_rec[1][2], (n_rec + 16) * sizeof(ST)));
                w0[1] = (uint64_t *)h->ar_rec[1][0].p; w1[1] = (uint64_t *)h->ar_rec[1][1].p; st[1] = (ST *)h->ar_rec[1][2].p;
            }
            const uint64_t p_lo = pre ? b_lo * nb2 : 0, p_n = pre ? (uint64_t)bps * nb2 : n_l2;
            CHK((multisplit_level<ST, true>(h, l2_start + p_lo, l2_cnt + p_lo, (uint32_t)p_n, 1, n_rec, w0[0], w1[0], st[0], w0[1],
                                            w1[1], st[1], top - SK_BUCKET_BITS, nb3, b_start + p_lo * nb3, b_cnt + p_lo * nb3,
                                            ms_scpre, ms_cmat, ms_offs, fb3)));
            where = 1;
        }
    } else {
        HIPCHK(h, hipMemcpyAsync(b_start, c1_start, (size_t)nb1 * 8, hipMemcpyDeviceToDevice, h->stream));
        HIPCHK(h, hipMemcpyAsync(b_cnt, c1_cnt, (size_t)nb1 * 8, hipMemcpyDeviceToDevice, h->stream));
    }
    h->stats.ms_partition = t_part.stop();
    h->stats.n_buckets = n_buckets;
    *out = SkPartition{b_start, b_cnt, n_buckets, where, l1, l2 > 0 ? nb2 : 1, fb2, l2_pow, nb3, fb3, est_distinct, n_inst, n_edge_inst};
    return DBG_OK;
}

static int resolve_counts_in(dbg *h) {
    if (!h->resolve_count) return DBG_OK;
    uint64_t c[2] = {0, 0};
    HIPCHK(h, hipMemcpyAsync(c, h->d_scalars + SC_RESOLVE_COUNTS, 16, hipMemcpyDeviceToHost, h->stream));
    HIPCHK(h, hipStreamSynchronize(h->stream));
    h->resolve_direct_hits += c[0];
    h->resolve_keyed += c[1];
    return DBG_OK;
}

template <class ST, int CAP, class STI = ST>
static int sk_count_from_segments(dbg *h, int k, const uint64_t *seg_start, const uint64_t *seg_cnt, uint32_t n_seg,
                                  const uint64_t *host_cnt, uint64_t n_rec, uint64_t n_inst, uint64_t n_edge_inst,
                                  const uint64_t *in_w0, const uint64_t *in_w1, const ST *in_st, uint64_t *w0[2], uint64_t *w1[2],
                                  ST *st[2], uint64_t node_capacity_hint, int shard_bits, int my_shard,
                                  const Presplit *pre = nullptr, const ExtractSplit *xs = nullptr) {
    const int m = sk_m_for_k(k);
    unsigned long long *sc_dev = (unsigned long long *)h->d_scalars;
    uint64_t sc[8] = {0};
    auto estimate = [h, k](unsigned grid, const uint64_t *s_start, const uint64_t *s_cnt, uint32_t seg, const uint64_t *rw0,
                           const uint64_t *rw1, unsigned long long *set, uint64_t set_mask, unsigned long long *d_est) {
        hipLaunchKernelGGL(HIP_KERNEL_NAME(k_estimate_distinct<ST>), dim3(grid), dim3(256), 0, h->stream, s_start, s_cnt, seg, rw0,
                           rw1, k, set, set_mask, d_est);
    };
    const SkPartitionParams<decltype(estimate)> pp{SK_TARGET_DISTINCT<CAP>, DBG_L1_WIDE_FROM, true, true, estimate};
    SkPartition P;
    CHK((sk_partition<ST, STI, 0>(h, pp, seg_start, seg_cnt, n_seg, host_cnt, pre, xs, in_w0, in_w1, in_st, w0, w1, st, shard_bits,
                                  my_shard, n_rec, n_inst, n_edge_inst, &P)));
    n_inst = P.n_inst;
    n_edge_inst = P.n_edge_inst;
    uint64_t *const b_start = P.b_start, *const b_cnt = P.b_cnt;
    const uint64_t n_buckets = P.n_buckets;
    const int where = P.where;
    const double est_distinct = P.est_distinct;

    const uint64_t id_limit = (shard_bits && !h->wide_owner) ? (h->shard_node_limit ? h->shard_node_limit : (1ull << 29) - 16)
                                                             : 0xFFFFFFF0ull;
    const uint32_t id_tag = (shard_bits && !h->wide_owner) ? ((uint32_t)my_shard << 29) : 0u;
    const uint64_t node_cap_max = std::min<uint64_t>(n_inst, id_limit);
    const uint64_t edge_cap_max = std::min<uint64_t>(n_edge_inst + 16, 0xFFFFFFF0ull);
    uint64_t node_cap = node_capacity_hint ? std::min<uint64_t>(node_capacity_hint, id_limit) : node_cap_max;
    if (!node_capacity_hint && est_distinct > 0.0)
        node_cap = std::min<uint64_t>(node_cap_max, (uint64_t)(est_distinct * 1.2 * h->est_scale_pct / 100.0) +
                                                        (h->est_scale_pct == 100 ? (1u << 20) : 1024u));
    uint64_t edge_cap = std::min<uint64_t>(edge_cap_max, node_cap + node_cap / 4 + 16);
    auto ensure_node_arrays = [&]() -> int {
        CHK(buf_ensure(h, h->ar_node[0], node_cap * 8));
        CHK(buf_ensure(h, h->ar_node[sizeof(ST) == 8 ? 1 : 7], node_cap * sizeof(ST)));
        CHK(buf_ensure(h, h->ar_node[3], node_cap));
        h->d_keys = (uint64_t *)h->ar_node[0].p;
        h->d_stamps_st = h->ar_node[sizeof(ST) == 8 ? 1 : 7].p;
        h->stamps_st_bytes = (int)sizeof(ST);
        h->d_stamps = sizeof(ST) == 8 ? (uint64_t *)h->d_stamps_st : nullptr;
        h->d_flags = (uint8_t *)h->ar_node[3].p;
        h->nodes_in_arena = true;
        CHK(buf_ensure(h, h->ar_csr[3], (node_cap + 1) * 4));
        CHK(buf_ensure(h, h->ar_csr[1], edge_cap * 4));
        CHK(buf_ensure(h, h->ar_csr[2], edge_cap * 4));
        h->d_rowptr32 = (uint32_t *)h->ar_csr[3].p;
        h->d_col = (uint32_t *)h->ar_csr[1].p;
        h->d_ecnt = (uint32_t *)h->ar_csr[2].p;
        return DBG_OK;
    };
    uint64_t q_cap = n_rec + 1024;
    uint64_t *qk[2], *qm[2];
    uint32_t *qc[2];
    const uint64_t range_cap = n_buckets + 4096 + n_inst / (CAP / 4);
    CHK(buf_ensure(h, h->ar_misc[MISC_RANGES], range_cap * sizeof(SkRange)));
    SkRange *ranges = (SkRange *)h->ar_misc[MISC_RANGES].p;
    const uint64_t own_cnt = n_buckets >> shard_bits, own_lo = (uint64_t)my_shard * own_cnt;
    CHK(buf_ensure(h, h->ar_dir, (own_cnt + (range_cap - n_buckets)) * (CAP / 64) * sizeof(SkDirEnt)));
    SkDirEnt *dirs = (SkDirEnt *)h->ar_dir.p;
    bool use_count2 = CAP == 4096 && h->count_kernel >= 2 && !h->phase_limit && (sizeof(ST) == 4 || h->count_kernel_u64 >= 2);
    const bool use_count3 = use_count2 && ((sizeof(ST) == 8 && h->count_kernel_u64 == 3) || h->count_kernel == 3);
    int extra_attempts = 0;
    for (int attempt = 0; attempt < 3 + extra_attempts; ++attempt) {
        CHK(ensure_node_arrays());
        for (int set = 0; set < 2; ++set) {
            CHK(buf_ensure(h, h->ar_q[set][0], q_cap * 8));
            CHK(buf_ensure(h, h->ar_q[set][2], q_cap * 4));
            if (shard_bits || h->resolve_sorted) CHK(buf_ensure(h, h->ar_q[set][1], q_cap * 8));
            qk[set] = (uint64_t *)h->ar_q[set][0].p;
            qm[set] = (uint64_t *)h->ar_q[set][1].p;
            qc[set] = (uint32_t *)h->ar_q[set][2].p;
            if (!shard_bits && !h->resolve_sorted) break;
        }
        Timer t(h->stream);
        HIPCHK(h, hipMemsetAsync(h->d_scalars, 0, 64 * 8, h->stream));
        HIPCHK(h, hipMemsetAsync(ranges, 0, n_buckets * sizeof(SkRange), h->stream));
        HIPCHK(h, hipMemsetAsync(dirs, 0, own_cnt * (CAP / 64) * sizeof(SkDirEnt), h->stream));
        SkCountOut out{h->d_keys, h->d_stamps_st, h->d_flags, node_cap, h->d_rowptr32, h->d_col, h->d_ecnt, edge_cap,
                       qk[0], qc[0], q_cap, ranges, n_buckets, range_cap, dirs, own_lo, own_cnt, id_tag, sc_dev};
        uint32_t split_recs = 0;
        if (est_distinct > 0.0 && n_rec)
            split_recs = (uint32_t)std::min<double>(1e9, std::max<double>(64.0, (CAP * 0.80) / (est_distinct / (double)n_rec)));
        if (use_count2 && n_rec) {
            auto kern2 = use_count3 ? k_sk_count3<ST> : k_sk_count2<ST>;
            const size_t lds2 = use_count3 ? sizeof(Cnt3Lds<ST>) : sizeof(Cnt2Lds<ST>);
            HIPCHK(h, hipFuncSetAttribute((const void *)kern2, hipFuncAttributeMaxDynamicSharedMemorySize, (int)lds2));
            int n_cu = 256;
            (void)hipDeviceGetAttribute(&n_cu, hipDeviceAttributeMultiprocessorCount, h->device);
            const unsigned grid = (unsigned)std::min<uint64_t>(n_buckets, (uint64_t)n_cu);
            SkCount2Args a2{out, b_start, b_cnt, w0[where], w1[where], (const void *)st[where], n_buckets, split_recs, k};
            SkCount2Args *d_a2 = (SkCount2Args *)(h->d_scalars + SC_DESCRIPTOR);
            static_assert(sizeof(SkCount2Args) <= (SK2_QUERY_CURSOR - SC_DESCRIPTOR) * 8, "the query cursor sits behind the descriptor");
            HIPCHK(h, hipMemcpyAsync(d_a2, &a2, sizeof(a2), hipMemcpyHostToDevice, h->stream));
            HIPCHK(h, hipMemsetAsync(h->d_scalars + SK2_QUERY_CURSOR, 0, 8, h->stream));
            hipLaunchKernelGGL(kern2, dim3(grid), dim3(Cnt2Cfg<ST>::NT), lds2, h->stream, (const SkCount2Args *)d_a2);
            HIPCHK(h, hipGetLastError());
        }
        auto kern = k_sk_count<ST, CAP>;
        const size_t lds = sizeof(CntLds<ST, CAP>);
        HIPCHK(h, hipFuncSetAttribute((const void *)kern, hipFuncAttributeMaxDynamicSharedMemorySize, (int)lds));
        if (n_rec && !use_count2) {
            int n_cu = 256;
            (void)hipDeviceGetAttribute(&n_cu, hipDeviceAttributeMultiprocessorCount, h->device);
            constexpr int NT = CntCfg<ST, CAP>::NT;
            const uint64_t per_cu = std::max<uint64_t>(1, std::min<uint64_t>(2048 / NT, (160 * 1024) / lds));
            const unsigned grid = (unsigned)std::min<uint64_t>(n_buckets, (uint64_t)n_cu * per_cu);
            static_assert(sizeof(SkCountOut) <= 64 * 8, "descriptor slot");
            SkCountOut *d_out = (SkCountOut *)(h->d_scalars + SC_DESCRIPTOR);
            HIPCHK(h, hipMemcpyAsync(d_out, &out, sizeof(out), hipMemcpyHostToDevice, h->stream));
            hipLaunchKernelGGL(kern, dim3(grid), dim3(NT), lds, h->stream, b_start, b_cnt, w0[where], w1[where],
                               st[where], k, m, n_buckets, (const SkCountOut *)d_out, split_recs, h->phase_limit);
            HIPCHK(h, hipGetLastError());
        }
        h->stats.count_launches = n_rec ? (uint64_t)(attempt + 1) : 0;
        HIPCHK(h, hipMemcpyAsync(sc, h->d_scalars, 64, hipMemcpyDeviceToHost, h->stream));
        uint64_t q2 = 0;
        if (use_count2 && n_rec) HIPCHK(h, hipMemcpyAsync(&q2, h->d_scalars + SK2_QUERY_CURSOR, 8, hipMemcpyDeviceToHost, h->stream));
        h->stats.ms_count = t.stop();
        if (use_count2 && n_rec) sc[5] = q2;
        if (h->phase_limit) { h->err = "ablation run (phase_limit set): timing only"; return DBG_E_ARG; }
        if (sc[0] & (STATUS_BUCKET_TOO_BIG | STATUS_RANGE_CAP)) break;
        bool again = false;
        if (use_count2 && (sc[0] & (STATUS_COUNTER16 | STATUS_INCONSISTENT))) {
            if ((sc[0] & STATUS_INCONSISTENT) && !(sc[0] & STATUS_COUNTER16)) { h->err = "internal: k_sk_count2 / k_sk_count3 counted a bucket's nodes, edges or queries inconsistently"; return DBG_E_HIP; }
            use_count2 = false;
            ++extra_attempts;
            again = true;
        }
        if ((sc[0] & STATUS_NODE_EDGE_CAP) && (node_cap < node_cap_max || edge_cap < edge_cap_max) && !node_capacity_hint) {
            node_cap = node_cap_max;
            edge_cap = edge_cap_max;
            again = true;
        }
        if ((sc[0] & STATUS_QUERY_CAP) && q_cap < n_edge_inst + 1024) { q_cap = n_edge_inst + 1024; again = true; }
        if (!again || attempt == 2 + extra_attempts) break;
    }
    if (sc[0] & STATUS_BUCKET_TOO_BIG) { h->err = "a bucket could not be split to fit the LDS table"; return DBG_E_CAPACITY; }
    if (sc[0] & STATUS_NODE_EDGE_CAP) { h->err = "node/edge capacity exceeded"; return DBG_E_CAPACITY; }
    if (sc[0] & (STATUS_RANGE_CAP | STATUS_QUERY_CAP)) { h->err = "range/query list overflow"; return DBG_E_CAPACITY; }
    h->n_nodes = sc[4] & 0xFFFFFFFFull;
    h->n_edges = sc[4] >> 32;
    {
        const uint32_t ne32 = (uint32_t)h->n_edges;
        HIPCHK(h, hipMemcpyAsync(h->d_rowptr32 + h->n_nodes, &ne32, 4, hipMemcpyHostToDevice, h->stream));
    }
    h->csr_built = true;
    h->dense_pending = true;
    uint64_t n_q = sc[5];
    const uint64_t n_ranges = n_buckets + sc[6];
    h->stats.n_queries = n_q;
    SkGeom geom{k, m, P.l1, P.nb2, P.fb2, P.l2_pow, P.nb3, P.fb3, shard_bits, my_shard, own_lo, own_cnt};

    {
        Timer t(h->stream);
        uint64_t root[2] = {0, n_q};
        int qset = 0;
        if (shard_bits && n_q) {
            hipLaunchKernelGGL(k_q_bucket, dim3(grid_for(n_q, 256)), dim3(256), 0, h->stream, qk[0], qm[0], n_q, k, m);
            HIPCHK(h, hipGetLastError());
            CHK(buf_ensure(h, h->ar_misc[MISC_QUERY_SEGS], 512 * 16 + 16));
            uint64_t *q_seg = (uint64_t *)h->ar_misc[MISC_QUERY_SEGS].p;
            const int nsh = 1 << shard_bits;
            HIPCHK(h, hipMemcpyAsync(q_seg, root, 16, hipMemcpyHostToDevice, h->stream));
            uint64_t *o_start = q_seg + 2, *o_cnt = o_start + nsh;
            CHK((multisplit_level<uint32_t, true>(h, q_seg, q_seg + 1, 1, 1, n_q, qk[0], qm[0], qc[0], qk[1], qm[1], qc[1],
                                                  40 + SK_BUCKET_BITS - shard_bits, nsh, o_start, o_cnt, h->ar_misc[MISC_MS_SCPRE],
                                                  h->ar_misc[MISC_MS_CMAT], h->ar_misc[MISC_MS_OFFS])));
            ShardState &sh = shard_of(h);
            sh.q_start.assign(nsh, 0);
            sh.q_cnt.assign(nsh, 0);
            HIPCHK(h, hipMemcpyAsync(sh.q_start.data(), o_start, (size_t)nsh * 8, hipMemcpyDeviceToHost, h->stream));
            HIPCHK(h, hipMemcpyAsync(sh.q_cnt.data(), o_cnt, (size_t)nsh * 8, hipMemcpyDeviceToHost, h->stream));
            HIPCHK(h, hipStreamSynchronize(h->stream));
            CHK(buf_ensure(h, h->ar_shard[0], n_q * 8));
            CHK(buf_ensure(h, h->ar_shard[3], n_q * 4));
            HIPCHK(h, hipMemcpyAsync(h->ar_shard[0].p, qk[1], n_q * 8, hipMemcpyDeviceToDevice, h->stream));
            HIPCHK(h, hipMemcpyAsync(h->ar_shard[3].p, qc[1], n_q * 4, hipMemcpyDeviceToDevice, h->stream));
            root[0] = sh.q_start[my_shard];
            root[1] = sh.q_cnt[my_shard];
            sh.n_remote = n_q - root[1];
            sh.q_cnt[my_shard] = 0;
            n_q = root[1];
            qset = 1;
        }
        const uint64_t *q_meta = nullptr;
        if (!shard_bits && h->resolve_sorted && (n_q >= (1u << 20) || (h->resolve_sorted == 2 && n_q))) {
            hipLaunchKernelGGL(k_q_bucket, dim3(grid_for(n_q, 256)), dim3(256), 0, h->stream, qk[0], qm[0], n_q, k, m);
            HIPCHK(h, hipGetLastError());
            CHK(buf_ensure(h, h->ar_misc[MISC_QUERY_SEGS], 1024 * 16 + 16));
            uint64_t *q_seg = (uint64_t *)h->ar_misc[MISC_QUERY_SEGS].p;
            HIPCHK(h, hipMemcpyAsync(q_seg, root, 16, hipMemcpyHostToDevice, h->stream));
            uint64_t *o_start = q_seg + 2, *o_cnt = o_start + 512;
            CHK((multisplit_level<uint32_t, true>(h, q_seg, q_seg + 1, 1, 1, n_q, qk[0], qm[0], qc[0], qk[1], qm[1], qc[1],
                                                  40 + SK_BUCKET_BITS - 9, 512, o_start, o_cnt, h->ar_misc[MISC_MS_SCPRE], h->ar_misc[MISC_MS_CMAT],
                                                  h->ar_misc[MISC_MS_OFFS])));
            qset = 1;
            q_meta = qm[1];
        }
        if (n_q) {
            const bool direct = !shard_bits && h->resolve_direct;
            auto resolver = direct ? k_succ_resolve<CAP, true, false> : k_succ_resolve<CAP, false, false>;
// ... 46 lines not shown
    const uint64_t tile_first = all_tiles * (uint64_t)part / (uint64_t)n_parts;
    const uint64_t tiles = all_tiles * (uint64_t)(part + 1) / (uint64_t)n_parts - tile_first;
    const bool reg_kernel = (w >= 20 && w <= 51) && !h->extract_generic;
    const uint32_t n_wg = (uint32_t)std::min<uint64_t>(std::max<uint64_t>(tiles, 1), reg_kernel ? 2048 : 1024);
    CHK(buf_ensure(h, h->ar_misc[MISC_SEGMENTS], (uint64_t)n_wg * 4 * 8));
    uint64_t *seg_start = (uint64_t *)h->ar_misc[MISC_SEGMENTS].p, *seg_cnt = seg_start + n_wg, *seg_nk = seg_cnt + n_wg, *seg_ne = seg_nk + n_wg;
    std::vector<uint64_t> hseg((size_t)n_wg * 4);
    uint64_t n_rec = 0;
    Timer t(h->stream);
    const uint64_t tiles_per_wg = (tiles + n_wg - 1) / n_wg;
    const double density = std::min(1.0, 2.6 / (double)(w + 1) + 1.3 * (double)(h->n_reads + 1) / (double)(h->n_bytes + 1) + 0.01);
    uint64_t seg_cap = (uint64_t)((double)(tiles_per_wg * TILE) * density) + 256;
    for (int attempt = 0; attempt < 2; ++attempt) {
        const uint64_t rec_cap = seg_cap * n_wg;
        for (int set = 0; set < 2; ++set) {
            CHK(buf_ensure(h, h->ar_rec[set][0], rec_cap * 8));
            CHK(buf_ensure(h, h->ar_rec[set][1], rec_cap * 8));
            CHK(buf_ensure(h, h->ar_rec[set][2], rec_cap * sizeof(ST)));
            w0[set] = (uint64_t *)h->ar_rec[set][0].p;
            w1[set] = (uint64_t *)h->ar_rec[set][1].p;
            st[set] = (ST *)h->ar_rec[set][2].p;
        }
        for (uint32_t g = 0; g < n_wg; ++g) hseg[g] = (uint64_t)g * seg_cap;
        HIPCHK(h, hipMemcpyAsync(seg_start, hseg.data(), (size_t)n_wg * 8, hipMemcpyHostToDevice, h->stream));
        HIPCHK(h, hipMemsetAsync(seg_cnt, 0, (size_t)n_wg * 3 * 8, h->stream));
        HIPCHK(h, hipMemsetAsync(h->d_scalars, 0, 64 * 8, h->stream));
        if (tiles && reg_kernel) {
#define DBG_WEXW_CASE(W_) case W_: hipLaunchKernelGGL(HIP_KERNEL_NAME(k_wsk_extract_w<ST, W_>), dim3(n_wg), dim3(256), 0, h->stream, \
                                                       h->d_bases, h->n_bytes, h->d_startbits, tiles, w0[0], w1[0], st[0], seg_cap, seg_cnt, \
                                                       seg_nk, seg_ne, sc_dev, tile_first); break;
            switch (w) {
                DBG_WEXW_CASE(20) DBG_WEXW_CASE(21) DBG_WEXW_CASE(22) DBG_WEXW_CASE(23) DBG_WEXW_CASE(24) DBG_WEXW_CASE(25)
                DBG_WEXW_CASE(26) DBG_WEXW_CASE(27) DBG_WEXW_CASE(28) DBG_WEXW_CASE(29) DBG_WEXW_CASE(30) DBG_WEXW_CASE(31)
                DBG_WEXW_CASE(32) DBG_WEXW_CASE(33) DBG_WEXW_CASE(34) DBG_WEXW_CASE(35) DBG_WEXW_CASE(36) DBG_WEXW_CASE(37)
                DBG_WEXW_CASE(38) DBG_WEXW_CASE(39) DBG_WEXW_CASE(40) DBG_WEXW_CASE(41) DBG_WEXW_CASE(42) DBG_WEXW_CASE(43)
                DBG_WEXW_CASE(44) DBG_WEXW_CASE(45) DBG_WEXW_CASE(46) DBG_WEXW_CASE(47) DBG_WEXW_CASE(48) DBG_WEXW_CASE(49)
                DBG_WEXW_CASE(50) DBG_WEXW_CASE(51)
                default: break;
            }
#undef DBG_WEXW_CASE
        } else if (tiles) {
            auto ekern = k_wsk_extract<ST>;
            HIPCHK(h, hipFuncSetAttribute((const void *)ekern, hipFuncAttributeMaxDynamicSharedMemorySize, (int)sizeof(WSkLds)));
            hipLaunchKernelGGL(ekern, dim3(n_wg), dim3(WSK_NT), sizeof(WSkLds), h->stream, h->d_bases, h->n_bytes,
                               h->d_startbits, k, tiles, w0[0], w1[0], st[0], seg_cap, seg_cnt, seg_nk, seg_ne, sc_dev, tile_first);
        }
        HIPCHK(h, hipGetLastError());
        HIPCHK(h, hipMemcpyAsync(sc, h->d_scalars, 8, hipMemcpyDeviceToHost, h->stream));
        HIPCHK(h, hipMemcpyAsync(hseg.data(), seg_start, (size_t)n_wg * 4 * 8, hipMemcpyDeviceToHost, h->stream));
        HIPCHK(h, hipStreamSynchronize(h->stream));
        if (sc[0] & STATUS_BAD_BASE) { h->err = "reads hold a byte outside ACGT"; return DBG_E_ALPHABET; }
        if (!(sc[0] & STATUS_SEGMENT_FULL)) break;
        if (attempt == 1) { h->err = "super-k-mer record buffer overflow"; return DBG_E_CAPACITY; }
        seg_cap = tiles_per_wg * TILE;
    }
    h->n_kmer_inst = h->n_edge_inst = 0;
    for (uint32_t g = 0; g < n_wg; ++g) {
        n_rec += hseg[n_wg + g];
        h->n_kmer_inst += hseg[2 * n_wg + g];
        h->n_edge_inst += hseg[3 * n_wg + g];
    }
    h->host_seg_cnt.assign(hseg.begin() + n_wg, hseg.begin() + 2 * (size_t)n_wg);
    h->stats.ms_extract = t.stop();
    h->stats.n_records = n_rec;
    *pk_out = pk; *seg_start_out = seg_start; *seg_cnt_out = seg_cnt; *n_seg_out = n_wg; *n_rec_out = n_rec;
    return DBG_OK;
}

template <class ST, class STI>
static int wsk_count(dbg *h, int k, const uint64_t *pk, const uint64_t *seg_start, const uint64_t *seg_cnt, uint32_t n_seg,
                     const uint64_t *host_cnt, uint64_t n_rec, uint64_t n_inst, uint64_t n_edge_inst, const uint64_t *in_w0,
                     const uint64_t *in_w1, const ST *in_st, uint64_t *w0[2], uint64_t *w1[2], ST *st[2], int shard_bits, int my_shard,
                     const Presplit *pre) {
    const int m = SK_MAX_M, w = k - m + 1;
    unsigned long long *sc_dev = (unsigned long long *)h->d_scalars;
    uint64_t sc[8] = {0};
    constexpr double TARGET_DISTINCT = 1000.0;
    constexpr int L1_WIDE_FROM = 18;
    constexpr int sthi = (sizeof(STI) == 4 && sizeof(ST) == 8) ? WREC_ST_HI : 0;
    auto estimate = [h, k, pk](unsigned grid, const uint64_t *s_start, const uint64_t *s_cnt, uint32_t seg, const uint64_t *rw0,
                               const uint64_t *rw1, unsigned long long *set, uint64_t set_mask, unsigned long long *d_est) {
        hipLaunchKernelGGL(k_wsk_estimate, dim3(grid), dim3(256), 0, h->stream, s_start, s_cnt, seg, rw0, rw1, k, pk, set, set_mask, d_est);
    };
    const SkPartitionParams<decltype(estimate)> pp{TARGET_DISTINCT, L1_WIDE_FROM, false, false, estimate};
    SkPartition P;
    CHK((sk_partition<ST, STI, sthi>(h, pp, seg_start, seg_cnt, n_seg, host_cnt, pre, nullptr, in_w0, in_w1, in_st, w0, w1, st,
                                     shard_bits, my_shard, n_rec, n_inst, n_edge_inst, &P)));
    uint64_t *const b_start = P.b_start, *const b_cnt = P.b_cnt;
    const uint64_t n_buckets = P.n_buckets;
    const int where = P.where;
    const double est_distinct = P.est_distinct;
    CHK(buf_ensure(h, h->ar_wide[2], (n_rec + 1) * 32));
    uint4 *rec_b = (uint4 *)h->ar_wide[2].p;
    {
        Timer t(h->stream);
        if (n_rec)
            hipLaunchKernelGGL(k_wsk_gather, dim3(grid_for(n_rec, 256)), dim3(256), 0, h->stream, w0[where], w1[where], n_rec, pk, k, rec_b);
        HIPCHK(h, hipGetLastError());
        h->stats.ms_compact = t.stop();
    }
    if (pre) {
        uint64_t tot_len = 0, tot_succ = 0;
        CHK(reduce_sum(h, n_rec, WRecLenAt{w1[where]}, &tot_len));
        CHK(reduce_sum(h, n_rec, WRecSuccAt{w1[where]}, &tot_succ));
        n_inst = tot_len;
        n_edge_inst = tot_len - n_rec + tot_succ;
        h->n_kmer_inst = n_inst;
        h->n_edge_inst = n_edge_inst;
    }
    const uint64_t id_limit = (shard_bits && !h->wide_owner) ? (h->shard_node_limit ? h->shard_node_limit : (1ull << 29) - 16)
                                                             : 0xFFFFFFF0ull;
    const uint32_t id_tag = (shard_bits && !h->wide_owner) ? ((uint32_t)my_shard << 29) : 0u;
    const uint64_t node_cap_max = std::min<uint64_t>(n_inst, id_limit);
    const uint64_t edge_cap_max = std::min<uint64_t>(n_edge_inst + 16, 0xFFFFFFF0ull);
    uint64_t node_cap = node_cap_max;
    if (est_distinct > 0.0)
        node_cap = std::min<uint64_t>(node_cap_max, (uint64_t)(est_distinct * 1.2 * h->est_scale_pct / 100.0) +
                                                        (h->est_scale_pct == 100 ? (1u << 20) : 1024u));
    uint64_t edge_cap = std::min<uint64_t>(edge_cap_max, node_cap + node_cap / 4 + 16);
    uint64_t q_cap = 2 * n_rec + 1024;
    const uint64_t own_cnt = n_buckets >> shard_bits, own_lo = (uint64_t)my_shard * own_cnt;
    const uint64_t range_cap = n_buckets + 4096 + n_inst / (WCAP / 4);
    CHK(buf_ensure(h, h->ar_misc[MISC_RANGES], range_cap * sizeof(SkRange)));
    SkRange *ranges = (SkRange *)h->ar_misc[MISC_RANGES].p;
    CHK(buf_ensure(h, h->ar_dir, (own_cnt + (range_cap - n_buckets)) * (WCAP / 64) * sizeof(SkDirEnt)));
    SkDirEnt *dirs = (SkDirEnt *)h->ar_dir.p;
    uint64_t *q_lo = nullptr, *q_hi = nullptr;
    uint32_t *q_col = nullptr;
    for (int attempt = 0; attempt < 3; ++attempt) {
        CHK(buf_ensure(h, h->ar_node[0], node_cap * 8));
        CHK(buf_ensure(h, h->ar_wide[5], node_cap * 8));
        CHK(buf_ensure(h, h->ar_node[sizeof(ST) == 8 ? 1 : 7], node_cap * sizeof(ST)));
        CHK(buf_ensure(h, h->ar_node[3], node_cap));
        CHK(buf_ensure(h, h->ar_csr[3], (node_cap + 1) * 4));
        CHK(buf_ensure(h, h->ar_csr[1], edge_cap * 4));
        CHK(buf_ensure(h, h->ar_csr[2], edge_cap * 4));
        CHK(buf_ensure(h, h->ar_q[0][0], q_cap * 8));
        CHK(buf_ensure(h, h->ar_q[0][1], q_cap * 8));
        CHK(buf_ensure(h, h->ar_q[0][2], q_cap * 4));
        h->d_keys = (uint64_t *)h->ar_node[0].p;
        h->d_keys_hi = (uint64_t *)h->ar_wide[5].p;
        h->d_stamps_st = h->ar_node[sizeof(ST) == 8 ? 1 : 7].p;
        h->stamps_st_bytes = (int)sizeof(ST);
        h->d_stamps = sizeof(ST) == 8 ? (uint64_t *)h->d_stamps_st : nullptr;
        h->d_flags = (uint8_t *)h->ar_node[3].p;
        h->nodes_in_arena = true;
        h->d_rowptr32 = (uint32_t *)h->ar_csr[3].p;
        h->d_col = (uint32_t *)h->ar_csr[1].p;
        h->d_ecnt = (uint32_t *)h->ar_csr[2].p;
        q_lo = (uint64_t *)h->ar_q[0][0].p; q_hi = (uint64_t *)h->ar_q[0][1].p; q_col = (uint32_t *)h->ar_q[0][2].p;
        Timer t(h->stream);
        HIPCHK(h, hipMemsetAsync(h->d_scalars, 0, 64 * 8, h->stream));
        HIPCHK(h, hipMemsetAsync(ranges, 0, n_buckets * sizeof(SkRange), h->stream));
        HIPCHK(h, hipMemsetAsync(dirs, 0, own_cnt * (WCAP / 64) * sizeof(SkDirEnt), h->stream));
        WSkCountOut out{h->d_keys, h->d_keys_hi, h->d_stamps_st, h->d_flags, node_cap, h->d_rowptr32, h->d_col, h->d_ecnt, edge_cap,
                        q_lo, q_hi, q_col, q_cap, ranges, n_buckets, range_cap, dirs, own_lo, own_cnt, sc_dev, id_tag};
        auto kern = k_wsk_count<ST>;
        size_t lds = sizeof(WCntLds<ST>);
        if constexpr (sizeof(ST) == 4) {
            if (h->wcount_kernel == 2) { kern = k_wsk_count2<ST>; lds = sizeof(WCnt2Lds); }
        }
        HIPCHK(h, hipFuncSetAttribute((const void *)kern, hipFuncAttributeMaxDynamicSharedMemorySize, (int)lds));
        if (n_rec) {
            int n_cu = 256;
            (void)hipDeviceGetAttribute(&n_cu, hipDeviceAttributeMultiprocessorCount, h->device);
            const unsigned grid = (unsigned)std::min<uint64_t>(n_buckets, (uint64_t)n_cu);
            uint32_t split_recs = 0;
            if (est_distinct > 0.0) split_recs = (uint32_t)std::min<double>(1e9, std::max<double>(16.0, (WCAP * 0.80) / (est_distinct / (double)n_rec)));
            static_assert(sizeof(WSkCountOut) <= 64 * 8, "descriptor slot");
            WSkCountOut *d_out = (WSkCountOut *)(h->d_scalars + SC_DESCRIPTOR);
            HIPCHK(h, hipMemcpyAsync(d_out, &out, sizeof(out), hipMemcpyHostToDevice, h->stream));
            hipLaunchKernelGGL(kern, dim3(grid), dim3(WCNT_NT), lds, h->stream, b_start, b_cnt, w0[where], w1[where], st[where],
                               (const uint4 *)rec_b, k, n_buckets, (const WSkCountOut *)d_out, split_recs);
            HIPCHK(h, hipGetLastError());
        }
        h->stats.count_launches = n_rec ? (uint64_t)(attempt + 1) : 0;
        HIPCHK(h, hipMemcpyAsync(sc, h->d_scalars, 64, hipMemcpyDeviceToHost, h->stream));
        h->stats.ms_count = t.stop();
        if (sc[0] & (STATUS_BUCKET_TOO_BIG | STATUS_RANGE_CAP | STATUS_COUNTER16 | STATUS_INCONSISTENT)) break;
        bool again = false;
        if ((sc[0] & STATUS_NODE_EDGE_CAP) && (node_cap < node_cap_max || edge_cap < edge_cap_max)) { node_cap = node_cap_max; edge_cap = edge_cap_max; again = true; }
        if ((sc[0] & STATUS_QUERY_CAP) && q_cap < n_edge_inst + 1024) { q_cap = n_edge_inst + 1024; again = true; }
// ... 852 lines not shown
}

static void multipass_free(dbg *h) {
    MultiPass *mp = (MultiPass *)h->multipass;
    if (!mp) return;
    for (auto *o : mp->col_owner) if (o) (void)hipFreeAsync(o, h->stream);
    for (auto *o : mp->pflags) if (o) (void)hipFree(o);
    for (dbg *sub : mp->part) {
        if (!sub) continue;
        if (mp->n_passes == 1 && mp->n_virtual <= 8 && !h->spare_part && !h->dropping_parts) { free_build(sub); h->spare_part = sub; }
        else dbg_destroy(sub);
    }
    delete mp;
    h->multipass = nullptr;
}

static void drop_spare_part(dbg *h) {
    if (!h->spare_part) return;
    dbg_destroy(h->spare_part);
    h->spare_part = nullptr;
    h->arena_freed = true;
}

static int multipass_starts(dbg *h, uint64_t *total) {
    MultiPass *mp = (MultiPass *)h->multipass;
    *total = 0;
    for (dbg *sub : mp->part) {
        uint64_t t = 0;
        if (sub->n_nodes) CHK(reduce_sum(h, sub->n_nodes, FlagSet{sub->d_flags, DBG_F_INDEG, 0}, &t));
        *total += t;
    }
    return DBG_OK;
}

__global__ __launch_bounds__(256) void k_apply_part(const uint32_t *__restrict__ qcol, const uint32_t *__restrict__ ans,
                                                    uint64_t n, uint8_t owner, uint32_t *col, uint8_t *col_owner,
                                                    unsigned long long *scalars) {
    uint64_t i = (uint64_t)blockIdx.x * blockDim.x + threadIdx.x;
    if (i >= n) return;
    const uint32_t a = ans[i];
    if (a == NO_NODE) { atomicOr(&scalars[0], STATUS_REMOTE_UNRESOLVED); return; }
    col[qcol[i]] = a;
    col_owner[qcol[i]] = owner;
}

template <class ST, class STI>
static int multipass_parts(dbg *h, int k, int n_virtual, int v_first, int n_passes, int n_senders, const uint64_t *grp_cnt,
                           const uint64_t *sender_off, const uint64_t *stamp_add, const uint64_t *in_w0,
                           const uint64_t *in_w1, const STI *in_st, const uint64_t *pk = nullptr) {
    int shard_bits = 0;
    while ((1 << shard_bits) < n_virtual) ++shard_bits;
    const int bps = 512 / n_virtual;
    const int own_groups = bps * n_passes;
    MultiPass *mp = new MultiPass();
    h->multipass = mp;
    mp->n_passes = n_passes;
    mp->n_virtual = n_virtual;
    mp->v_first = v_first;
    mp->part.assign(n_passes, nullptr);
    mp->col_owner.assign(n_passes, nullptr);
    mp->pflags.assign(n_passes, nullptr);
    mp->base.assign(n_passes + 1, 0);
    const int w = k - sk_m_for_k(k) + 1;
    double ms_count = 0, ms_part = h->stats.ms_partition, ms_succ = 0;
    uint64_t n_buckets = 0, n_queries = 0;
    std::vector<uint64_t> p_cnt((size_t)n_senders * bps), p_off(n_senders);
    for (int p = 0; p < n_passes; ++p) {
        dbg *sub = nullptr;
        const bool reused = n_passes == 1 && h->spare_part;
        if (reused) { sub = h->spare_part; h->spare_part = nullptr; }
        else sub = new (std::nothrow) dbg();
        if (!sub) return DBG_E_NOMEM;
        mp->part[p] = sub;
        sub->device = h->device;
        sub->stream = h->stream;
        sub->borrowed_stream = true;
        sub->wide_owner = true;
        sub->bucket_bits = h->bucket_bits;
        sub->count_kernel = h->count_kernel;
        sub->count_kernel_u64 = h->count_kernel_u64;
        sub->wcount_kernel = h->wcount_kernel;
        sub->resolve_sorted = h->resolve_sorted;
        sub->resolve_direct = h->resolve_direct;
        sub->resolve_count = h->resolve_count;
        sub->target_distinct = h->target_distinct;
        sub->est_scale_pct = h->est_scale_pct;
        if (!sub->d_scalars) HIPCHK(h, hipMalloc((void **)&sub->d_scalars, 128 * sizeof(uint64_t)));
        sub->k = k;
        uint64_t n_rec_p = 0;
        for (int r = 0; r < n_senders; ++r) {
            uint64_t before = 0;
            for (int g = 0; g < p * bps; ++g) before += grp_cnt[(size_t)r * own_groups + g];
            p_off[r] = sender_off[r] + before;
            for (int b = 0; b < bps; ++b) {
                p_cnt[(size_t)r * bps + b] = grp_cnt[(size_t)r * own_groups + (size_t)p * bps + b];
                n_rec_p += p_cnt[(size_t)r * bps + b];
            }
        }
        uint64_t *pw0[2] = {nullptr, nullptr}, *pw1[2] = {nullptr, nullptr};
        ST *pst[2] = {nullptr, nullptr};
        CHK(buf_ensure(sub, sub->ar_rec[0][0], (n_rec_p + 16) * 8));
        CHK(buf_ensure(sub, sub->ar_rec[0][1], (n_rec_p + 16) * 8));
        CHK(buf_ensure(sub, sub->ar_rec[0][2], (n_rec_p + 16) * sizeof(ST)));
        pw0[0] = (uint64_t *)sub->ar_rec[0][0].p; pw1[0] = (uint64_t *)sub->ar_rec[0][1].p; pst[0] = (ST *)sub->ar_rec[0][2].p;
        ShardState &sh = shard_of(sub);
        sh.n_shards = n_virtual; sh.my_shard = v_first + p; sh.shard_bits = shard_bits; sh.k = k; sh.n_remote = 0;
        sh.q_start.assign(n_virtual, 0);
        sh.q_cnt.assign(n_virtual, 0);
        Presplit pre;
        pre.n_senders = n_senders;
        pre.counts = p_cnt.data();
        pre.recv_off = p_off.data();
        pre.stamp_add = stamp_add;
        pre.in_st = in_st;
        int rc = DBG_OK;
        if (n_rec_p && pk) {
            rc = wsk_count<ST, STI>(sub, k, pk, nullptr, nullptr, 0, nullptr, n_rec_p, n_rec_p * (uint64_t)w, n_rec_p * (uint64_t)w, in_w0,
                                    in_w1, (const ST *)nullptr, pw0, pw1, pst, shard_bits, v_first + p, &pre);
        } else if (n_rec_p)
            rc = sk_count_from_segments<ST, 4096, STI>(sub, k, nullptr, nullptr, 0, nullptr, n_rec_p, n_rec_p * (uint64_t)w, n_rec_p * (uint64_t)w,
                                                       in_w0, in_w1, (const ST *)nullptr, pw0, pw1, pst, 0, shard_bits, v_first + p, &pre);
        if (rc != DBG_OK) { h->err = "pass " + std::to_string(p) + ": " + sub->err; return rc; }
        if (n_rec_p && n_passes > 1) {
            const uint64_t own_cnt = sub->sk_n_buckets >> shard_bits;
            rc = part_compact(sub, (own_cnt + (sub->sk_n_ranges - sub->sk_n_buckets)) * (4096 / 64));
            if (rc != DBG_OK) { h->err = "pass " + std::to_string(p) + ": " + sub->err; return rc; }
        }
        mp->base[p + 1] = mp->base[p] + sub->n_nodes;
        if (sub->n_edges) {
            HIPCHK(h, hipMallocAsync((void **)&mp->col_owner[p], sub->n_edges, h->stream));
            HIPCHK(h, hipMemsetAsync(mp->col_owner[p], v_first + p, sub->n_edges, h->stream));
        }
        (void)reused;
        ms_count += sub->stats.ms_count; ms_part += sub->stats.ms_partition; ms_succ += sub->stats.ms_succ;
        n_buckets += sub->stats.n_buckets >> shard_bits; n_queries += sub->stats.n_queries;
        h->stats.count_launches += sub->stats.count_launches;
    }
    {
        Timer t(h->stream);
        uint64_t max_q = 0;
        for (int p = 0; p < n_passes; ++p) {
            ShardState &sh = shard_of(mp->part[p]);
            for (int q = 0; q < n_passes; ++q) if (q != p) max_q = std::max(max_q, sh.q_cnt[v_first + q]);
        }
        CHK(buf_ensure(h, h->ar_shard[2], (max_q + 16) * 4));
        uint32_t *ans = (uint32_t *)h->ar_shard[2].p;
        HIPCHK(h, hipMemsetAsync(h->d_scalars, 0, 8, h->stream));
        for (int p = 0; p < n_passes; ++p) {
            dbg *sub = mp->part[p];
            ShardState &sh = shard_of(sub);
            const uint64_t *keys = (const uint64_t *)sub->ar_shard[0].p;
            const uint32_t *qcol = (const uint32_t *)sub->ar_shard[3].p;
            const uint64_t qw = pk ? 2 : 1;
            for (int q = 0; q < n_passes; ++q) {
                const int vq = v_first + q;
                if (q == p || !sh.q_cnt[vq]) continue;
                if (!mp->part[q]->n_nodes) { h->err = "part " + std::to_string(q) + " is empty and cannot own a successor"; return DBG_E_HIP; }
                int rc = dbg_shard_answer(mp->part[q], keys + qw * sh.q_start[vq], sh.q_cnt[vq], ans);
                if (rc != DBG_OK) { h->err = "part " + std::to_string(q) + ": " + mp->part[q]->err; return rc; }
                hipLaunchKernelGGL(k_apply_part, dim3(grid_for(sh.q_cnt[vq], 256)), dim3(256), 0, h->stream, qcol + sh.q_start[vq],
                                   ans, sh.q_cnt[vq], (uint8_t)vq, sub->d_col, mp->col_owner[p], (unsigned long long *)h->d_scalars);
            }
            if (n_virtual == n_passes) {
                buf_free(sub, sub->ar_shard[0]);
                buf_free(sub, sub->ar_shard[3]);
            }
// ... 1010 lines not shown
```

py-debruijn_amd/csrc/dbg_sk.h:

```cpp
#pragma once
#include <cstddef>
#include "dbg_device.h"
#include "dbg_dir.h"
#include "dbg_minwin.h"

namespace dbgk {

constexpr int SK_MAX_M = 13;
constexpr int SK_BUCKET_BITS = 22;
constexpr int SK_META_BITS = 28;

__host__ __device__ inline int sk_m_for_k(int k) { return k < SK_MAX_M ? k : SK_MAX_M; }

__host__ __device__ inline uint32_t fmix32(uint32_t x) {
    x ^= x >> 16; x *= 0x85EBCA6Bu;
    x ^= x >> 13; x *= 0xC2B2AE35u;
    x ^= x >> 16;
    return x;
}
__device__ inline uint32_t bucket_hash22(uint32_t mmer) { return fmix32(mmer * 0x9E3779B1u + 0x7F4A7C15u) >> (32 - SK_BUCKET_BITS); }

__device__ inline uint32_t kmer_bucket22(uint64_t kmer, int k, int m) {
    const int w = k - m + 1;
    const uint32_t mmask = (uint32_t)((1ull << (2 * m)) - 1);
// ... 505 lines not shown
                rk[i] = atomicAdd(&s.hist[ms_child(r1[i], shift, nb, fbits)], 1u);
            }
        }
        __syncthreads();
        MS_TICK(2);
        {
            constexpr int EPT = MS_MAX_NB / MS_NT;
            const int b0 = threadIdx.x * EPT;
            uint32_t h4[EPT];
            uint64_t sum = 0;
#pragma unroll
            for (int j = 0; j < EPT; ++j) { h4[j] = (b0 + j < nb) ? s.hist[b0 + j] : 0; sum += h4[j]; }
            uint64_t tot;
            uint32_t ex = (uint32_t)block_exscan<MS_NT / 64>(sum, &tot);
#pragma unroll
            for (int j = 0; j < EPT; ++j) { if (b0 + j < nb) s.start[b0 + j] = ex; ex += h4[j]; }
        }
        __syncthreads();
        MS_TICK(3);
#pragma unroll
        for (int i = 0; i < CH / MS_NT; ++i) {
            const int q = i * MS_NT + threadIdx.x;
            if (q < n) {
                const uint32_t b = ms_child(r1[i], shift, nb, fbits);
                const uint32_t d = s.start[b] + rk[i];
                s.w0[d] = r0[i];
                s.w1[d] = r1[i];
                if (HAS_ST) s.st[d] = rs[i];
            }
        }
        __syncthreads();
        MS_TICK(4);
        for (int q = threadIdx.x; q < n; q += MS_NT) {
            const uint64_t x1 = s.w1[q];
            const uint32_t b = ms_child(x1, shift, nb, fbits);
            const uint64_t g = s.run[b] + (q - s.start[b]);
            out_w0[g] = s.w0[q];
            out_w1[g] = x1;
            if (HAS_ST) out_st[g] = s.st[q];
        }
        __syncthreads();
        MS_TICK(5);
        for (int b = threadIdx.x; b < nb; b += MS_NT) s.run[b] += s.hist[b];
        __syncthreads();
        MS_TICK(6);
    }
#ifdef DBG_MS_PROF
    if (threadIdx.x == 0) {
        for (int i = 0; i < 7; ++i) atomicAdd(&g_ms_prof[i], prof_[i]);
        atomicAdd(&g_ms_prof[7], 1ull);
    }
#endif
}


template <class ST>
__global__ __launch_bounds__(256) void k_estimate_distinct(const uint64_t *__restrict__ b_start,
                                                           const uint64_t *__restrict__ b_cnt, uint32_t bucket,
                                                           const uint64_t *__restrict__ rec_w0,
                                                           const uint64_t *__restrict__ rec_w1, int k,
                                                           unsigned long long *set, uint64_t set_mask,
                                                           unsigned long long *out ) {
    const uint64_t beg = b_start[bucket], n = b_cnt[bucket];
    uint64_t inst = 0, fresh = 0;
    for (uint64_t r = (uint64_t)blockIdx.x * blockDim.x + threadIdx.x; r < n; r += (uint64_t)gridDim.x * blockDim.x) {
        const uint64_t w0 = rec_w0[beg + r], w1 = rec_w1[beg + r];
        const uint64_t hi = w1 & (~0ull << SK_META_BITS);
        const int len = (int)((w1 >> 1) & 31) + 1;
        for (int i = 0; i < len; ++i) {
            const uint64_t kmer = (i ? (w0 << (2 * i)) | (hi >> (64 - 2 * i)) : w0) >> (64 - 2 * k);
            ++inst;
            uint64_t slot = mix64(kmer) & set_mask;
            for (uint64_t probe = 0; probe <= set_mask; ++probe) {
                unsigned long long cur = set[slot];
                if (cur == EMPTY_KEY) {
                    cur = atomicCAS(&set[slot], EMPTY_KEY, (unsigned long long)kmer);
                    if (cur == EMPTY_KEY) { ++fresh; break; }
                }
                if (cur == kmer) break;
                slot = (slot + 1) & set_mask;
            }
        }
    }
    inst = wave_sum_u64(inst);
    fresh = wave_sum_u64(fresh);
    if ((threadIdx.x & 63) == 0) {
        if (inst) atomicAdd(&out[0], (unsigned long long)inst);
        if (fresh) atomicAdd(&out[1], (unsigned long long)fresh);
    }
}

struct SkRange {
    uint32_t bucket;
    uint32_t mask, val;
    uint32_t node_cnt;
    uint64_t node_base;
    uint32_t next;
    uint32_t pad;
};

__device__ inline uint32_t fold32(uint64_t kmer) { return (uint32_t)kmer * 0x9E3779B1u ^ (uint32_t)(kmer >> 32) * 0x85EBCA77u; }
__device__ inline uint32_t sub_hash(uint64_t kmer) { return fmix32(fold32(kmer) ^ 0x27D4EB2Fu); }
__device__ inline uint32_t slot_hash(uint64_t kmer) {
    const uint32_t lo = (uint32_t)kmer, hi = (uint32_t)(kmer >> 32);
    return (lo ^ (hi << 11) ^ (hi >> 7) ^ (lo >> 15)) * 0x9E3779B1u;
}
template <int CAP>
__device__ inline uint32_t slot_of(uint64_t kmer) {
    static_assert(CAP == 2048 || CAP == 4096, "table size");
    return slot_hash(kmer) >> (CAP == 4096 ? 20 : 21);
}

template <class ST, int CAP>
struct CntCfg {
    #ifdef DBG_CNT_PROF
    static constexpr int QBUF = CAP == 4096 ? (sizeof(ST) == 8 ? 624 : 768) : 400;
#else
    static constexpr int QBUF = CAP == 4096 ? (sizeof(ST) == 8 ? 640 : 768) : 400;
#endif
    static constexpr int NT = CAP == 4096 ? 1024 : 512;
};
constexpr int CNT_STACK = 24;
constexpr int CNT_PROBE_LIMIT = 1024;

template <class ST, int CAP>
struct CntLds {
    static constexpr int CNT_QBUF = CntCfg<ST, CAP>::QBUF;
    unsigned long long keys[CAP];
    uint32_t cnt[CAP * 4];
    ST stamp[CAP];
    uint16_t list[CAP];
    uint16_t eoff[CAP];
    unsigned long long q_key[CNT_QBUF];
    unsigned long long q_meta[CNT_QBUF];
    ST st_stage[CNT_QBUF];
    uint32_t stk_mask[CNT_STACK], stk_val[CNT_STACK];
    int stk_n;
    uint32_t overflow, n_local , n_q, fail, n_flat;
    unsigned long long gbase, qbase, ebase, ri;
    unsigned long long dir_mask[CAP / 64];
    uint16_t dir_base[CAP / 64];
#ifdef DBG_CNT_PROF
    unsigned long long prof[64];
#endif
};

__device__ inline uint64_t rec_window(uint64_t w0, uint64_t hi, int i) {
    return (w0 << (2 * i)) | ((hi >> 1) >> (63 - 2 * i));
}

template <int CAP>
__device__ inline int lds_find(const unsigned long long *keys, uint64_t key) {
    uint32_t slot = slot_of<CAP>(key);
#pragma unroll 16
    for (int probe = 0; probe < CAP; ++probe) {
        const unsigned long long cur = keys[slot];
        if (cur == key) return (int)slot;
        if (cur == EMPTY_KEY) return -1;
        slot = (slot + 1) & (CAP - 1);
    }
    return -1;
}


struct SkCountOut {
    uint64_t *keys;
// ... 609 lines not shown
```

Measured before the change: 59.99 billion.

## Overlap distinct-count estimate with level-1 scatter on a side stream

Result: slower. 58.60 billion (-2.3%).

```diff
diff --git a/py-debruijn_amd/_dbg.py b/py-debruijn_amd/_dbg.py
--- a/py-debruijn_amd/_dbg.py
+++ b/py-debruijn_amd/_dbg.py
@@ -67,7 +67,8 @@
     _fields_ = [("src", C.c_void_p), ("contigs", C.c_void_p), ("n", C.c_uint64)]
 
 
-COUNTERS = ("extract_presplit_fallbacks", "extract_presplit_rehists", "resolve_direct_hits", "resolve_keyed")
+COUNTERS = ("extract_presplit_fallbacks", "extract_presplit_rehists", "partition_ahead_estimates", "resolve_direct_hits",
+            "resolve_keyed")
 
 
 class DbgError(RuntimeError):
diff --git a/py-debruijn_amd/csrc/dbg_hip.hip b/py-debruijn_amd/csrc/dbg_hip.hip
--- a/py-debruijn_amd/csrc/dbg_hip.hip
+++ b/py-debruijn_amd/csrc/dbg_hip.hip
@@ -164,6 +164,20 @@
     bool arena_freed = false;
     std::vector<uint64_t> host_seg_cnt;
     std::vector<uint64_t> host_scpre;
+    int partition_ahead = 1;
+    uint64_t partition_ahead_estimates = 0;
+    hipStream_t side = nullptr;
+    hipEvent_t ev_children = nullptr, ev_side = nullptr, ev_part[2] = {nullptr, nullptr};
+    bool part_time_pending = false;
+    uint64_t *pin_side = nullptr;
+    struct PinBuf {
+        void *p = nullptr;
+        uint64_t bytes = 0;
+        hipEvent_t busy = nullptr;
+        bool in_flight = false;
+    };
+    PinBuf pin_scpre[2], pin_seg;
+    int pin_scpre_turn = 0;
     uint64_t shard_node_limit = 0;
     bool partial_graph = false;
     uint64_t *d_btab = nullptr;
@@ -286,6 +300,56 @@
         (void)hipEventDestroy(b);
     }
 };
+
+constexpr uint64_t PIN_SIDE_WORDS = 2 + 1024;
+static int host_aux_ensure(dbg *h) {
+    if (h->pin_side) return DBG_OK;
+    if (!h->side) HIPCHK(h, hipStreamCreateWithFlags(&h->side, hipStreamNonBlocking));
+    for (hipEvent_t *e : {&h->ev_children, &h->ev_side})
+        if (!*e) HIPCHK(h, hipEventCreateWithFlags(e, hipEventDisableTiming));
+    for (hipEvent_t *e : {&h->ev_part[0], &h->ev_part[1]})
+        if (!*e) HIPCHK(h, hipEventCreate(e));
+    HIPCHK(h, hipHostMalloc((void **)&h->pin_side, PIN_SIDE_WORDS * 8, hipHostMallocDefault));
+    return DBG_OK;
+}
+static void host_aux_free(dbg *h) {
+    if (h->side) { (void)hipStreamSynchronize(h->side); (void)hipStreamDestroy(h->side); h->side = nullptr; }
+    for (hipEvent_t *e : {&h->ev_children, &h->ev_side, &h->ev_part[0], &h->ev_part[1]})
+        if (*e) { (void)hipEventDestroy(*e); *e = nullptr; }
+    if (h->pin_side) { (void)hipHostFree(h->pin_side); h->pin_side = nullptr; }
+    for (dbg::PinBuf *b : {&h->pin_scpre[0], &h->pin_scpre[1], &h->pin_seg}) {
+        if (b->busy) (void)hipEventDestroy(b->busy);
+        if (b->p) (void)hipHostFree(b->p);
+        *b = dbg::PinBuf{};
+    }
+}
+
+static int pin_ensure(dbg *h, dbg::PinBuf &b, uint64_t bytes) {
+    if (!b.busy) HIPCHK(h, hipEventCreateWithFlags(&b.busy, hipEventDisableTiming));
+    if (b.in_flight) { HIPCHK(h, hipEventSynchronize(b.busy)); b.in_flight = false; }
+    if (b.bytes >= bytes) return DBG_OK;
+    if (b.p) (void)hipHostFree(b.p);
+    b.p = nullptr;
+    b.bytes = 0;
+    const uint64_t want = std::max<uint64_t>(4096, bytes + bytes / 2);
+    HIPCHK(h, hipHostMalloc(&b.p, want, hipHostMallocDefault));
+    b.bytes = want;
+    return DBG_OK;
+}
+static int pin_upload(dbg *h, dbg::PinBuf &b, void *dst, uint64_t bytes) {
+    HIPCHK(h, hipMemcpyAsync(dst, b.p, bytes, hipMemcpyHostToDevice, h->stream));
+    HIPCHK(h, hipEventRecord(b.busy, h->stream));
+    b.in_flight = true;
+    return DBG_OK;
+}
+
+static void partition_time_in(dbg *h) {
+    if (!h->part_time_pending) return;
+    h->part_time_pending = false;
+    float ms = 0;
+    if (hipEventElapsedTime(&ms, h->ev_part[0], h->ev_part[1]) == hipSuccess) h->stats.ms_partition = ms;
+    else (void)hipGetLastError();
+}
 
 constexpr int SCAN_ITEMS = 16;
 constexpr int SCAN_TILE = 256 * SCAN_ITEMS;
@@ -1478,7 +1542,8 @@
     if (!h) return DBG_E_NOMEM;
     h->device = device;
     if (hipSetDevice(device) != hipSuccess || hipStreamCreate(&h->stream) != hipSuccess ||
-        hipMalloc((void **)&h->d_scalars, 128 * sizeof(uint64_t)) != hipSuccess) {
+        hipMalloc((void **)&h->d_scalars, 128 * sizeof(uint64_t)) != hipSuccess || host_aux_ensure(h) != DBG_OK) {
+        host_aux_free(h);
         delete h;
         return DBG_E_HIP;
     }
@@ -1519,6 +1584,7 @@
     dev_free(h->d_scalars);
     delete (ShardState *)h->shard_state;
     (void)hipStreamSynchronize(h->stream);
+    host_aux_free(h);
     if (!h->borrowed_stream) (void)hipStreamDestroy(h->stream);
     delete h;
 }
@@ -2285,6 +2351,7 @@
     if (n == "stamp64" && (value == 0 || value == 1)) { h->stamp64 = (int)value; return DBG_OK; }
     if (n == "resolve_sorted" && value >= 0 && value <= 2) { h->resolve_sorted = (int)value; return DBG_OK; }
     if (n == "resolve_direct" && (value == 0 || value == 1)) { h->resolve_direct = (int)value; return DBG_OK; }
+    if (n == "partition_ahead" && (value == 0 || value == 1)) { h->partition_ahead = (int)value; return DBG_OK; }
     if (n == "resolve_count" && (value == 0 || value == 1)) { h->resolve_count = (int)value; return DBG_OK; }
     if (n == "wcount_kernel" && (value == 1 || value == 2)) { h->wcount_kernel = (int)value; return DBG_OK; }
     if (n == "count_kernel_u64" && value >= 1 && value <= 3) { h->count_kernel_u64 = (int)value; return DBG_OK; }
@@ -3168,6 +3235,7 @@
     const std::string n(name);
     if (n == "extract_presplit_rehists") { *out = h->presplit_rehists; return DBG_OK; }
     if (n == "extract_presplit_fallbacks") { *out = h->presplit_fallbacks; return DBG_OK; }
+    if (n == "partition_ahead_estimates") { *out = h->partition_ahead_estimates; return DBG_OK; }
     if (n == "resolve_direct_hits") { *out = h->resolve_direct_hits; return DBG_OK; }
     if (n == "resolve_keyed") { *out = h->resolve_keyed; return DBG_OK; }
     h->err = "unknown counter: " + n;
@@ -3389,22 +3457,23 @@
                             uint64_t *out_w0, uint64_t *out_w1, ST *out_st, int shift, int nb, uint64_t *c_start,
                             uint64_t *c_cnt, dbg::Buf &b_scpre, dbg::Buf &b_cmat, dbg::Buf &b_offs, int fbits = 0,
                             const uint64_t *seg_add = nullptr, unsigned long long *d_sums = nullptr,
-                            const uint64_t *host_cnt = nullptr, const uint32_t *ready_cmat = nullptr) {
+                            const uint64_t *host_cnt = nullptr, const uint32_t *ready_cmat = nullptr,
+                            hipEvent_t children_done = nullptr) {
     CHK(buf_ensure(h, b_scpre, (uint64_t)(n_seg + 1) * 8));
     uint64_t *sc_pre = (uint64_t *)b_scpre.p;
     uint64_t nsc = 0;
-    if (ready_cmat) {
-        std::vector<uint64_t> &pre = h->host_scpre;
-        pre.resize((size_t)n_seg + 1);
-        for (uint32_t i = 0; i <= n_seg; ++i) pre[i] = i;
-        nsc = n_seg;
-        HIPCHK(h, hipMemcpyAsync(sc_pre, pre.data(), pre.size() * 8, hipMemcpyHostToDevice, h->stream));
-    } else if (host_cnt) {
-        std::vector<uint64_t> &pre = h->host_scpre;
-        pre.resize((size_t)n_seg + 1);
-        for (uint32_t i = 0; i < n_seg; ++i) { pre[i] = nsc; nsc += (host_cnt[i] + MS_SC - 1) / MS_SC; }
-        pre[n_seg] = nsc;
-        HIPCHK(h, hipMemcpyAsync(sc_pre, pre.data(), pre.size() * 8, hipMemcpyHostToDevice, h->stream));
+    if (ready_cmat || host_cnt) {
+        dbg::PinBuf &pin = h->pin_scpre[h->pin_scpre_turn ^= 1];
+        CHK(pin_ensure(h, pin, ((uint64_t)n_seg + 1) * 8));
+        uint64_t *pre = (uint64_t *)pin.p;
+        if (ready_cmat) {
+            for (uint32_t i = 0; i <= n_seg; ++i) pre[i] = i;
+            nsc = n_seg;
+        } else {
+            for (uint32_t i = 0; i < n_seg; ++i) { pre[i] = nsc; nsc += (host_cnt[i] + MS_SC - 1) / MS_SC; }
+            pre[n_seg] = nsc;
+        }
+        CHK(pin_upload(h, pin, sc_pre, ((uint64_t)n_seg + 1) * 8));
     } else {
         CHK(exclusive_scan(h, n_seg, CeilDiv{p_cnt, (uint64_t)MS_SC}, sc_pre, &nsc));
         HIPCHK(h, hipMemcpyAsync(sc_pre + n_seg, &nsc, 8, hipMemcpyHostToDevice, h->stream));
@@ -3430,6 +3499,7 @@
     const uint64_t n_child = (uint64_t)(n_seg / spg) * nb;
     hipLaunchKernelGGL(k_ms_children, dim3(grid_for(n_child, 256)), dim3(256), 0, h->stream, P, offs, nb, total, c_start,
                        c_cnt);
+    if (children_done) HIPCHK(h, hipEventRecord(children_done, h->stream));
     if (nsc) {
         auto kern = k_ms_scatter<ST, HAS_ST, STI, STHI>;
         const size_t lds = sizeof(MsLds<ST>);
@@ -3500,7 +3570,7 @@
         sk_provisional_bits(h, h->n_bytes > cut ? h->n_bytes - cut : 0, 1.0, xs->target, 0, false, DBG_L1_WIDE_FROM, &T_guess, &ps_l1);
         if (ps_l1 < f0) ps_l1 = 0;
     }
-    std::vector<uint64_t> hseg;
+    uint64_t *hseg = nullptr;
     uint64_t *seg_start = nullptr, *seg_cnt = nullptr, *seg_nk = nullptr, *seg_ne = nullptr;
     uint32_t *ps_cmat = nullptr;
     uint64_t n_rec = 0;
@@ -3508,7 +3578,10 @@
     for (int attempt = 0; attempt < 3; ++attempt) {
         CHK(buf_ensure(h, h->ar_misc[MISC_SEGMENTS], (n_seg * 2 + (uint64_t)n_wg * 2) * 8));
         seg_start = (uint64_t *)h->ar_misc[MISC_SEGMENTS].p; seg_cnt = seg_start + n_seg; seg_nk = seg_cnt + n_seg; seg_ne = seg_nk + n_wg;
-        hseg.assign((size_t)(n_seg * 2 + (uint64_t)n_wg * 2), 0);
+        const uint64_t hseg_n = n_seg * 2 + (uint64_t)n_wg * 2;
+        CHK(pin_ensure(h, h->pin_seg, (hseg_n + 1) * 8));
+        hseg = (uint64_t *)h->pin_seg.p;
+        memset(hseg, 0, (size_t)(hseg_n + 1) * 8);
         if (f0 && ps_l1) {
             CHK(buf_ensure(h, h->ar_misc[MISC_MS_CMAT], n_seg * 4 << (ps_l1 - f0)));
             ps_cmat = (uint32_t *)h->ar_misc[MISC_MS_CMAT].p;
@@ -3523,7 +3596,7 @@
             st[set] = (ST *)h->ar_rec[set][2].p;
         }
         for (uint64_t g = 0; g < n_seg; ++g) hseg[g] = g * seg_cap;
-        HIPCHK(h, hipMemcpyAsync(seg_start, hseg.data(), (size_t)n_seg * 8, hipMemcpyHostToDevice, h->stream));
+        CHK(pin_upload(h, h->pin_seg, seg_start, n_seg * 8));
         HIPCHK(h, hipMemsetAsync(seg_cnt, 0, (size_t)(n_seg + (uint64_t)n_wg * 2) * 8, h->stream));
         HIPCHK(h, hipMemsetAsync(h->d_scalars, 0, 64 * 8, h->stream));
         if (tiles) {
@@ -3551,10 +3624,12 @@
                                    seg_ne, sc_dev, tile_first);
             HIPCHK(h, hipGetLastError());
         }
-        HIPCHK(h, hipMemcpyAsync(sc, h->d_scalars, 8, hipMemcpyDeviceToHost, h->stream));
-        HIPCHK(h, hipMemcpyAsync(hseg.data() + n_seg, seg_cnt, (size_t)(n_seg + (uint64_t)n_wg * 2) * 8, hipMemcpyDeviceToHost,
+        HIPCHK(h, hipMemcpyAsync(hseg + hseg_n, h->d_scalars, 8, hipMemcpyDeviceToHost, h->stream));
+        HIPCHK(h, hipMemcpyAsync(hseg + n_seg, seg_cnt, (size_t)(n_seg + (uint64_t)n_wg * 2) * 8, hipMemcpyDeviceToHost,
                                  h->stream));
         HIPCHK(h, hipStreamSynchronize(h->stream));
+        h->pin_seg.in_flight = false;
+        sc[0] = hseg[hseg_n];
         if (sc[0] & STATUS_BAD_BASE) { h->err = "reads hold a byte outside ACGT"; return DBG_E_ALPHABET; }
         if (!(sc[0] & STATUS_SEGMENT_FULL)) break;
         if (f0) {
@@ -3576,7 +3651,7 @@
     }
     h->stats.ms_extract = t.stop();
     h->stats.n_records = n_rec;
-    h->host_seg_cnt.assign(hseg.begin() + n_seg, hseg.begin() + 2 * (size_t)n_seg);
+    h->host_seg_cnt.assign(hseg + n_seg, hseg + 2 * (size_t)n_seg);
     if (xs) { xs->f0 = f0; xs->n_wg = n_wg; xs->l1 = ps_l1; xs->cmat = ps_l1 ? ps_cmat : nullptr; }
     *seg_start_out = seg_start;
     *seg_cnt_out = seg_cnt;
@@ -3601,6 +3676,7 @@
     bool probe_first_owned;
     bool sum_instances;
     Est estimate;
+    int ahead_k = 0;
 };
 
 struct SkPartition {
@@ -3631,7 +3707,23 @@
     int where = 0;
     double est_distinct = 0.0;
     const int top = 6 + SK_BUCKET_BITS;
-    Timer t_part(h->stream);
+    const bool want_estimate = auto_T && l1 >= 9 && n_rec;
+    const uint32_t probe_bucket = (pp.probe_first_owned && shard_bits) ? (uint32_t)my_shard << (l1 - shard_bits) : 0u;
+    uint64_t set_cap = 1024;
+    unsigned long long *set = nullptr, *const d_est = (unsigned long long *)(h->d_scalars + SC_ESTIMATE);
+    if (want_estimate) {
+        const uint64_t inst_bucket = (uint64_t)((double)n_inst * own / nb1) * 2 + 1024;
+        while (set_cap < inst_bucket * 2) set_cap <<= 1;
+        CHK(buf_ensure(h, h->ar_misc[MISC_ESTIMATE_SET], set_cap * 8));
+        set = (unsigned long long *)h->ar_misc[MISC_ESTIMATE_SET].p;
+    }
+    CHK(host_aux_ensure(h));
+    const bool l1_presplit = !pre && xs && xs->f0 && l1 >= xs->f0;
+    const bool ahead = h->partition_ahead && l1_presplit && want_estimate && pp.ahead_k > 0;
+    uint64_t *const pin_est = h->pin_side, *const pin_c1 = h->pin_side + 2;
+    bool side_pending = false;
+    HIPCHK(h, hipEventRecord(h->ev_part[0], h->stream));
+    h->part_time_pending = false;
     const int bps = pre ? nb1 >> shard_bits : 0;
     const uint64_t b_lo = pre ? (uint64_t)my_shard * bps : 0;
     uint64_t *ps_start = nullptr, *ps_cnt = nullptr, *ps_add = nullptr;
@@ -3659,31 +3751,48 @@
             if (xs->l1 != l1) ++h->presplit_rehists;
             CHK((multisplit_level<ST, true>(h, seg_start, seg_cnt, n_seg, xs->n_wg, n_rec, in_w0, in_w1, in_st, w0[1], w1[1], st[1],
                                             top - l1, nb1 >> xs->f0, c1_start, c1_cnt, ms_scpre, ms_cmat, ms_offs, 0, nullptr, nullptr,
-                                            host_cnt, xs->l1 == l1 ? xs->cmat : nullptr)));
+                                            host_cnt, xs->l1 == l1 ? xs->cmat : nullptr, h->ev_children)));
         } else {
             CHK((multisplit_level<ST, true>(h, seg_start, seg_cnt, n_seg, n_seg, n_rec, in_w0, in_w1, in_st, w0[1], w1[1], st[1],
-                                            top - l1, nb1, c1_start, c1_cnt, ms_scpre, ms_cmat, ms_offs, 0, nullptr, nullptr, host_cnt)));
+                                            top - l1, nb1, c1_start, c1_cnt, ms_scpre, ms_cmat, ms_offs, 0, nullptr, nullptr, host_cnt,
+                                            nullptr, h->ev_children)));
         }
         where = 1;
-    }
-    if (auto_T && l1 >= 9 && n_rec) {
-        const uint32_t probe_bucket = (pp.probe_first_owned && shard_bits) ? (uint32_t)my_shard << (l1 - shard_bits) : 0u;
-        const uint64_t inst_bucket = (uint64_t)((double)n_inst * own / nb1) * 2 + 1024;
-        uint64_t set_cap = 1024;
-        while (set_cap < inst_bucket * 2) set_cap <<= 1;
-        CHK(buf_ensure(h, h->ar_misc[MISC_ESTIMATE_SET], set_cap * 8));
-        unsigned long long *set = (unsigned long long *)h->ar_misc[MISC_ESTIMATE_SET].p;
-        unsigned long long *d_est = (unsigned long long *)(h->d_scalars + SC_ESTIMATE);
-        HIPCHK(h, hipMemsetAsync(set, 0xFF, set_cap * 8, h->stream));
-        HIPCHK(h, hipMemsetAsync(d_est, 0, 16, h->stream));
-        if (pre) {
-            for (int r = 0; r < pre->n_senders; ++r) pp.estimate(128u, ps_start, ps_cnt, (uint32_t)r, in_w0, in_w1, set, set_cap - 1, d_est);
+        HIPCHK(h, hipStreamWaitEvent(h->side, h->ev_children, 0));
+        if (ahead) {
+            const int f0 = xs->f0;
+            const uint32_t digit_mask = (uint32_t)(nb1 >> f0) - 1u;
+            HIPCHK(h, hipMemsetAsync(set, 0xFF, set_cap * 8, h->side));
+            HIPCHK(h, hipMemsetAsync(d_est, 0, 16, h->side));
+            hipLaunchKernelGGL(k_estimate_distinct_presplit, dim3(std::min<uint32_t>(xs->n_wg, 512u)), dim3(EST_NT), 0, h->side, seg_start,
+                               seg_cnt, (probe_bucket >> (l1 - f0)) * xs->n_wg, xs->n_wg, top - l1, digit_mask, probe_bucket & digit_mask,
+                               in_w0, in_w1, pp.ahead_k, set, set_cap - 1, d_est);
+            HIPCHK(h, hipGetLastError());
+            HIPCHK(h, hipMemcpyAsync(pin_est, d_est, 16, hipMemcpyDeviceToHost, h->side));
+            ++h->partition_ahead_estimates;
+        }
+        HIPCHK(h, hipMemcpyAsync(pin_c1, c1_cnt, (size_t)nb1 * 8, hipMemcpyDeviceToHost, h->side));
+        side_pending = true;
+    }
+    if (side_pending) HIPCHK(h, hipEventRecord(h->ev_side, h->side));
+    if (want_estimate) {
+        uint64_t est[2] = {0, 0};
+        if (ahead) {
+            HIPCHK(h, hipEventSynchronize(h->ev_side));
+            side_pending = false;
+            est[0] = pin_est[0];
+            est[1] = pin_est[1];
         } else {
-            pp.estimate(512u, c1_start, c1_cnt, probe_bucket, w0[1], w1[1], set, set_cap - 1, d_est);
-        }
-        uint64_t est[2] = {0, 0};
-        HIPCHK(h, hipMemcpyAsync(est, d_est, 16, hipMemcpyDeviceToHost, h->stream));
-        HIPCHK(h, hipStreamSynchronize(h->stream));
+            HIPCHK(h, hipMemsetAsync(set, 0xFF, set_cap * 8, h->stream));
+            HIPCHK(h, hipMemsetAsync(d_est, 0, 16, h->stream));
+            if (pre) {
+                for (int r = 0; r < pre->n_senders; ++r) pp.estimate(128u, ps_start, ps_cnt, (uint32_t)r, in_w0, in_w1, set, set_cap - 1, d_est);
+            } else {
+                pp.estimate(512u, c1_start, c1_cnt, probe_bucket, w0[1], w1[1], set, set_cap - 1, d_est);
+            }
+            HIPCHK(h, hipMemcpyAsync(est, d_est, 16, hipMemcpyDeviceToHost, h->stream));
+            HIPCHK(h, hipStreamSynchronize(h->stream));
+        }
         if (est[0]) {
             double distinct = (double)n_inst * own * (double)est[1] / (double)est[0];
             if (pre) {
@@ -3741,8 +3850,10 @@
                 h->n_edge_inst = n_edge_inst;
             }
         } else {
+            if (side_pending) { HIPCHK(h, hipEventSynchronize(h->ev_side)); side_pending = false; }
             CHK((multisplit_level<ST, true>(h, c1_start, c1_cnt, (uint32_t)nb1, 1, n_rec, w0[1], w1[1], st[1], w0[0], w1[0],
-                                            st[0], sh2, nb2, l2_start, l2_cnt, ms_scpre, ms_cmat, ms_offs, fb2)));
+                                            st[0], sh2, nb2, l2_start, l2_cnt, ms_scpre, ms_cmat, ms_offs, fb2, nullptr, nullptr,
+                                            pin_c1)));
         }
         where = 0;
         if (nb3 > 1) {
@@ -3762,7 +3873,9 @@
         HIPCHK(h, hipMemcpyAsync(b_start, c1_start, (size_t)nb1 * 8, hipMemcpyDeviceToDevice, h->stream));
         HIPCHK(h, hipMemcpyAsync(b_cnt, c1_cnt, (size_t)nb1 * 8, hipMemcpyDeviceToDevice, h->stream));
     }
-    h->stats.ms_partition = t_part.stop();
+    if (side_pending) HIPCHK(h, hipEventSynchronize(h->ev_side));
+    HIPCHK(h, hipEventRecord(h->ev_part[1], h->stream));
+    h->part_time_pending = true;
     h->stats.n_buckets = n_buckets;
     *out = SkPartition{b_start, b_cnt, n_buckets, where, l1, l2 > 0 ? nb2 : 1, fb2, l2_pow, nb3, fb3, est_distinct, n_inst, n_edge_inst};
     return DBG_OK;
@@ -3792,7 +3905,7 @@
         hipLaunchKernelGGL(HIP_KERNEL_NAME(k_estimate_distinct<ST>), dim3(grid), dim3(256), 0, h->stream, s_start, s_cnt, seg, rw0,
                            rw1, k, set, set_mask, d_est);
     };
-    const SkPartitionParams<decltype(estimate)> pp{SK_TARGET_DISTINCT<CAP>, DBG_L1_WIDE_FROM, true, true, estimate};
+    const SkPartitionParams<decltype(estimate)> pp{SK_TARGET_DISTINCT<CAP>, DBG_L1_WIDE_FROM, true, true, estimate, k};
     SkPartition P;
     CHK((sk_partition<ST, STI, 0>(h, pp, seg_start, seg_cnt, n_seg, host_cnt, pre, xs, in_w0, in_w1, in_st, w0, w1, st, shard_bits,
                                   my_shard, n_rec, n_inst, n_edge_inst, &P)));
@@ -3899,6 +4012,7 @@
         uint64_t q2 = 0;
         if (use_count2 && n_rec) HIPCHK(h, hipMemcpyAsync(&q2, h->d_scalars + SK2_QUERY_CURSOR, 8, hipMemcpyDeviceToHost, h->stream));
         h->stats.ms_count = t.stop();
+        partition_time_in(h);
         if (use_count2 && n_rec) sc[5] = q2;
         if (h->phase_limit) { h->err = "ablation run (phase_limit set): timing only"; return DBG_E_ARG; }
         if (sc[0] & (STATUS_BUCKET_TOO_BIG | STATUS_RANGE_CAP)) break;
@@ -4111,7 +4225,7 @@
                                const uint64_t *rw1, unsigned long long *set, uint64_t set_mask, unsigned long long *d_est) {
         hipLaunchKernelGGL(k_wsk_estimate, dim3(grid), dim3(256), 0, h->stream, s_start, s_cnt, seg, rw0, rw1, k, pk, set, set_mask, d_est);
     };
-    const SkPartitionParams<decltype(estimate)> pp{TARGET_DISTINCT, L1_WIDE_FROM, false, false, estimate};
+    const SkPartitionParams<decltype(estimate)> pp{TARGET_DISTINCT, L1_WIDE_FROM, false, false, estimate, 0};
     SkPartition P;
     CHK((sk_partition<ST, STI, sthi>(h, pp, seg_start, seg_cnt, n_seg, host_cnt, pre, nullptr, in_w0, in_w1, in_st, w0, w1, st,
                                      shard_bits, my_shard, n_rec, n_inst, n_edge_inst, &P)));
@@ -4127,6 +4241,7 @@
             hipLaunchKernelGGL(k_wsk_gather, dim3(grid_for(n_rec, 256)), dim3(256), 0, h->stream, w0[where], w1[where], n_rec, pk, k, rec_b);
         HIPCHK(h, hipGetLastError());
         h->stats.ms_compact = t.stop();
+        partition_time_in(h);
     }
     if (pre) {
         uint64_t tot_len = 0, tot_succ = 0;
@@ -5145,6 +5260,7 @@
         sub->wcount_kernel = h->wcount_kernel;
         sub->resolve_sorted = h->resolve_sorted;
         sub->resolve_direct = h->resolve_direct;
+        sub->partition_ahead = h->partition_ahead;
         sub->resolve_count = h->resolve_count;
         sub->target_distinct = h->target_distinct;
         sub->est_scale_pct = h->est_scale_pct;
diff --git a/py-debruijn_amd/csrc/dbg_sk.h b/py-debruijn_amd/csrc/dbg_sk.h
--- a/py-debruijn_amd/csrc/dbg_sk.h
+++ b/py-debruijn_amd/csrc/dbg_sk.h
@@ -611,6 +611,73 @@
             }
         }
     }
+    inst = wave_sum_u64(inst);
+    fresh = wave_sum_u64(fresh);
+    if ((threadIdx.x & 63) == 0) {
+        if (inst) atomicAdd(&out[0], (unsigned long long)inst);
+        if (fresh) atomicAdd(&out[1], (unsigned long long)fresh);
+    }
+}
+
+constexpr int EST_NT = 256, EST_ITEMS = 4;
+constexpr int EST_QUEUE = EST_NT * (EST_ITEMS + 1);
+__global__ __launch_bounds__(EST_NT) void k_estimate_distinct_presplit(const uint64_t *__restrict__ seg_start,
+                                                                       const uint64_t *__restrict__ seg_cnt, uint32_t first_seg,
+                                                                       uint32_t n_wg, int shift, uint32_t digit_mask, uint32_t digit,
+                                                                       const uint64_t *__restrict__ rec_w0,
+                                                                       const uint64_t *__restrict__ rec_w1, int k,
+                                                                       unsigned long long *set, uint64_t set_mask,
+                                                                       unsigned long long *out ) {
+    __shared__ uint64_t q_w0[EST_QUEUE], q_w1[EST_QUEUE];
+    __shared__ uint32_t q_n;
+    uint64_t inst = 0, fresh = 0;
+    auto insert = [&](uint64_t w0, uint64_t w1) {
+        const uint64_t hi = w1 & (~0ull << SK_META_BITS);
+        const int len = (int)((w1 >> 1) & 31) + 1;
+        for (int i = 0; i < len; ++i) {
+            const uint64_t kmer = (i ? (w0 << (2 * i)) | (hi >> (64 - 2 * i)) : w0) >> (64 - 2 * k);
+            ++inst;
+            uint64_t slot = mix64(kmer) & set_mask;
+            for (uint64_t probe = 0; probe <= set_mask; ++probe) {
+                unsigned long long cur = set[slot];
+                if (cur == EMPTY_KEY) {
+                    cur = atomicCAS(&set[slot], EMPTY_KEY, (unsigned long long)kmer);
+                    if (cur == EMPTY_KEY) { ++fresh; break; }
+                }
+                if (cur == kmer) break;
+                slot = (slot + 1) & set_mask;
+            }
+        }
+    };
+    if (threadIdx.x == 0) q_n = 0;
+    __syncthreads();
+    for (uint32_t wg = blockIdx.x; wg < n_wg; wg += gridDim.x) {
+        const uint64_t beg = seg_start[first_seg + wg], n = seg_cnt[first_seg + wg];
+        for (uint64_t c0 = 0; c0 < n; c0 += (uint64_t)EST_NT * EST_ITEMS) {
+#pragma unroll
+            for (int i = 0; i < EST_ITEMS; ++i) {
+                const uint64_t r = c0 + (uint64_t)i * EST_NT + threadIdx.x;
+                if (r < n) {
+                    const uint64_t w1 = rec_w1[beg + r];
+                    if (((uint32_t)(w1 >> shift) & digit_mask) == digit) {
+                        const uint32_t at = atomicAdd(&q_n, 1u);
+                        q_w0[at] = rec_w0[beg + r];
+                        q_w1[at] = w1;
+                    }
+                }
+            }
+            __syncthreads();
+            uint32_t have = q_n;
+            __syncthreads();
+            while (have >= (uint32_t)EST_NT) {
+                have -= EST_NT;
+                insert(q_w0[have + threadIdx.x], q_w1[have + threadIdx.x]);
+            }
+            if (threadIdx.x == 0) q_n = have;
+            __syncthreads();
+        }
+    }
+    if (threadIdx.x < q_n) insert(q_w0[threadIdx.x], q_w1[threadIdx.x]);
     inst = wave_sum_u64(inst);
     fresh = wave_sum_u64(fresh);
     if ((threadIdx.x & 63) == 0) {
```
